# Z2PackDev/TBmodels

Measured on AMD Instinct MI355X. Metric: k-points/sec (H(k)+eig) at N_orb=64, N_R=4096, higher is better.
Workload: dtype f64; 1 GPU; cfg2: dense N_orb=64 N_R=4096, 100000 random k-points per GPU, eigenval (H(k)+eig); kpoints_per_gpu=100000, collective=none, rccl_ranks=0, eigensolver=auto

## Files before the change

### include/tbk.h

```cpp
#ifndef TBK_H
#define TBK_H

#include <stdint.h>

#ifdef __cplusplus
extern "C" {
#endif

typedef struct tbk_model tbk_model;
typedef struct tbk_kdotp tbk_kdotp;
typedef struct tbk_comm tbk_comm;

typedef enum tbk_status {
    TBK_OK = 0,
    TBK_ERR_ARGUMENT = 1,
    TBK_ERR_DEVICE = 2,
    TBK_ERR_MEMORY = 3,
    TBK_ERR_NOT_FINITE = 4,
    TBK_ERR_NO_CONVERGENCE = 5
} tbk_status;

enum { TBK_EIG_AUTO = 0, TBK_EIG_WAVE = 1, TBK_EIG_ROCSOLVER = 2 };
enum {
    TBK_OPT_EIGENSOLVER = 1,
    TBK_OPT_K_CHUNK = 2,
    TBK_OPT_TIMING = 3,
    TBK_OPT_FOLD = 4
};

const char* tbk_version(void);
const char* tbk_last_error(void);
int tbk_device_count(int* count);


int tbk_model_create_dense(int device, int dim, int n_orb, int64_t n_r, const int32_t* R,
                           const double* hop, tbk_model** out);

int tbk_model_create_csr(int device, int dim, int n_orb, int64_t n_r, const int32_t* R,
                         const int64_t* r_ptr, const int32_t* row, const int32_t* col,
                         const double* val, tbk_model** out);

void tbk_model_destroy(tbk_model* m);
int tbk_model_set_option(tbk_model* m, int option, int64_t value);
int tbk_model_info(const tbk_model* m, int* device, int* dim, int* n_orb, int64_t* n_r,
                   int* is_sparse, int64_t* staged_bytes);
enum { TBK_CNT_EIGENVAL_CALLS = 0, TBK_CNT_FOLDED_CALLS = 1, TBK_CNT_FOLDED_KPOINTS = 2,
       TBK_CNT_LIBRARY_CALLS = 3,
       TBK_CNT_COUNT = 4 };
int tbk_model_counter(tbk_model* m, int counter, int64_t* value);


int tbk_hamilton(tbk_model* m, const double* k, int64_t nk, int convention, const double* pos,
                 double* H_out);

int tbk_eigenval(tbk_model* m, const double* k, int64_t nk, double* E_out);

int tbk_eigenval_multi(tbk_model* const* handles, int n_handles, const double* k, int64_t nk, double* E_out);
int tbk_hamilton_multi(tbk_model* const* handles, int n_handles, const double* k, int64_t nk, int convention,
                       const double* pos, double* H_out);

int tbk_hamilton_device(tbk_model* m, const double* d_k, int64_t nk, int convention,
                        const double* d_pos, double* d_H);
int tbk_eigenval_device(tbk_model* m, const double* d_k, int64_t nk, double* d_E);
int tbk_eigenval_device_hint(tbk_model* m, const double* d_k, const double* h_k, int64_t nk, double* d_E);
int tbk_eigenval_check(tbk_model* m);
int tbk_synchronize(tbk_model* m);

enum { TBK_REDUCE_AUTO = 0, TBK_REDUCE_ONE_STAGE = 1, TBK_REDUCE_TWO_STAGE = 2 };
int tbk_tridiagonal_reduce(int device, int n_orb, int64_t nk, const double* H, int method, double* d, double* e,
                           double* H_reduced);

int tbk_reduce_standalone(int device, int n_orb, int64_t nk, int reps, double* us_per_matrix);

int tbk_kdotp_create(int device, int dim, int n_orb, int64_t n_p, const int32_t* powers,
                     const double* coeffs, tbk_kdotp** out);
void tbk_kdotp_destroy(tbk_kdotp* m);
int tbk_kdotp_hamilton(tbk_kdotp* m, const double* k, int64_t nk, double* H_out);
int tbk_kdotp_eigenval(tbk_kdotp* m, const double* k, int64_t nk, double* E_out);
int tbk_kdotp_eigenval_multi(tbk_kdotp* const* handles, int n_handles, const double* k, int64_t nk, double* E_out);
int tbk_kdotp_hamilton_multi(tbk_kdotp* const* handles, int n_handles, const double* k, int64_t nk, double* H_out);

int tbk_kdotp_coefficients(tbk_model* m, const double* k0, int64_t n_p, const int32_t* powers,
                           const double* prefactor, double* coeffs_out);

int tbk_device_malloc(int device, int64_t bytes, void** d_ptr);
int tbk_device_free(int device, void* d_ptr);
int tbk_memcpy_h2d(int device, void* d_dst, const void* h_src, int64_t bytes);
int tbk_memcpy_d2h(int device, void* h_dst, const void* d_src, int64_t bytes);
int tbk_device_mem_info(int device, int64_t* free_bytes, int64_t* total_bytes);

enum { TBK_T_PHASE = 0, TBK_T_HK = 1, TBK_T_EIG = 2, TBK_T_QL = 3, TBK_T_COUNT = 4 };
int tbk_get_timing(tbk_model* m, double* ms, int64_t* launches, int reset);

int tbk_comm_unique_id(void* id128);
int tbk_comm_create(int device, int world_size, int rank, const void* id128, tbk_comm** out);
void tbk_comm_destroy(tbk_comm* c);
int tbk_comm_ranks(tbk_comm* c, int* count, int* rank);
int tbk_comm_allgather_f64(tbk_comm* c, tbk_model* m, const double* d_send, double* d_recv,
                           int64_t count);
int tbk_comm_allgather_f64_overlapped(tbk_comm* c, tbk_model* m, const double* d_send, double* d_recv,
                                      int64_t count, int slot);
int tbk_comm_wait_slot(tbk_comm* c, tbk_model* m, int slot);
int tbk_comm_synchronize(tbk_comm* c);
int tbk_comm_agree(tbk_comm* c, int status, double* verdict);
int tbk_comm_prepare_gather(tbk_comm* c, int n_orb, int64_t per);

int tbk_eigenval_device_gather(tbk_comm* c, tbk_model* m, const double* d_k, const double* h_k, int64_t nk, int64_t per,
                               int host_status, double* d_all, double* d_status_all);

int tbk_mfma_f64_peak(int device, double* tflops);

#ifdef __cplusplus
}
#endif
#endif
```

### tbmodels_amd/_lib.py

```python

import ctypes
import os

import numpy as np

_HERE = os.path.dirname(os.path.abspath(__file__))
LIB_PATH = os.environ.get("TBK_LIBTBK") or os.path.join(_HERE, "libtbk.so")

TBK_OK = 0
TBK_ERR_ARGUMENT = 1
TBK_ERR_DEVICE = 2
TBK_ERR_MEMORY = 3
TBK_ERR_NOT_FINITE = 4
TBK_ERR_NO_CONVERGENCE = 5

TBK_EIG_AUTO, TBK_EIG_WAVE, TBK_EIG_ROCSOLVER = 0, 1, 2
TBK_OPT_EIGENSOLVER, TBK_OPT_K_CHUNK, TBK_OPT_TIMING, TBK_OPT_FOLD = 1, 2, 3, 4
TBK_REDUCE_AUTO, TBK_REDUCE_ONE_STAGE, TBK_REDUCE_TWO_STAGE = 0, 1, 2
TBK_CNT_EIGENVAL_CALLS, TBK_CNT_FOLDED_CALLS, TBK_CNT_FOLDED_KPOINTS, TBK_CNT_LIBRARY_CALLS = 0, 1, 2, 3
TBK_T_PHASE, TBK_T_HK, TBK_T_EIG, TBK_T_QL, TBK_T_COUNT = 0, 1, 2, 3, 4
STAGE_NAMES = ("phase", "hk", "eig", "ql")

_c_int = ctypes.c_int
_c_i64 = ctypes.c_int64
_vp = ctypes.c_void_p
_pp = ctypes.POINTER(ctypes.c_void_p)

SIGNATURES = {
    "tbk_version": (ctypes.c_char_p, []),
    "tbk_last_error": (ctypes.c_char_p, []),
    "tbk_device_count": (_c_int, [ctypes.POINTER(_c_int)]),
    "tbk_model_create_dense": (_c_int, [_c_int, _c_int, _c_int, _c_i64, _vp, _vp, _pp]),
    "tbk_model_create_csr": (_c_int, [_c_int, _c_int, _c_int, _c_i64, _vp, _vp, _vp, _vp, _vp, _pp]),
    "tbk_model_destroy": (None, [_vp]),
    "tbk_model_set_option": (_c_int, [_vp, _c_int, _c_i64]),
    "tbk_model_info": (
        _c_int,
        [_vp, ctypes.POINTER(_c_int), ctypes.POINTER(_c_int), ctypes.POINTER(_c_int), ctypes.POINTER(_c_i64),
         ctypes.POINTER(_c_int), ctypes.POINTER(_c_i64)],
    ),
    "tbk_hamilton": (_c_int, [_vp, _vp, _c_i64, _c_int, _vp, _vp]),
    "tbk_eigenval": (_c_int, [_vp, _vp, _c_i64, _vp]),
    "tbk_eigenval_multi": (_c_int, [_vp, _c_int, _vp, _c_i64, _vp]),
    "tbk_hamilton_multi": (_c_int, [_vp, _c_int, _vp, _c_i64, _c_int, _vp, _vp]),
    "tbk_hamilton_device": (_c_int, [_vp, _vp, _c_i64, _c_int, _vp, _vp]),
    "tbk_eigenval_device": (_c_int, [_vp, _vp, _c_i64, _vp]),
    "tbk_eigenval_device_hint": (_c_int, [_vp, _vp, _vp, _c_i64, _vp]),
    "tbk_model_counter": (_c_int, [_vp, _c_int, ctypes.POINTER(_c_i64)]),
    "tbk_eigenval_check": (_c_int, [_vp]),
    "tbk_synchronize": (_c_int, [_vp]),
    "tbk_tridiagonal_reduce": (_c_int, [_c_int, _c_int, _c_i64, _vp, _c_int, _vp, _vp, _vp]),
    "tbk_reduce_standalone": (_c_int, [_c_int, _c_int, _c_i64, _c_int, ctypes.POINTER(ctypes.c_double)]),
    "tbk_kdotp_create": (_c_int, [_c_int, _c_int, _c_int, _c_i64, _vp, _vp, _pp]),
    "tbk_kdotp_destroy": (None, [_vp]),
    "tbk_kdotp_hamilton": (_c_int, [_vp, _vp, _c_i64, _vp]),
    "tbk_kdotp_eigenval": (_c_int, [_vp, _vp, _c_i64, _vp]),
    "tbk_kdotp_eigenval_multi": (_c_int, [_vp, _c_int, _vp, _c_i64, _vp]),
    "tbk_kdotp_hamilton_multi": (_c_int, [_vp, _c_int, _vp, _c_i64, _vp]),
    "tbk_kdotp_coefficients": (_c_int, [_vp, _vp, _c_i64, _vp, _vp, _vp]),
    "tbk_device_malloc": (_c_int, [_c_int, _c_i64, _pp]),
    "tbk_device_free": (_c_int, [_c_int, _vp]),
    "tbk_memcpy_h2d": (_c_int, [_c_int, _vp, _vp, _c_i64]),
    "tbk_memcpy_d2h": (_c_int, [_c_int, _vp, _vp, _c_i64]),
    "tbk_device_mem_info": (_c_int, [_c_int, ctypes.POINTER(_c_i64), ctypes.POINTER(_c_i64)]),
    "tbk_get_timing": (_c_int, [_vp, ctypes.POINTER(ctypes.c_double), ctypes.POINTER(_c_i64), _c_int]),
    "tbk_comm_unique_id": (_c_int, [_vp]),
    "tbk_comm_create": (_c_int, [_c_int, _c_int, _c_int, _vp, _pp]),
    "tbk_comm_destroy": (None, [_vp]),
    "tbk_comm_ranks": (_c_int, [_vp, ctypes.POINTER(_c_int), ctypes.POINTER(_c_int)]),
    "tbk_comm_allgather_f64": (_c_int, [_vp, _vp, _vp, _vp, _c_i64]),
    "tbk_comm_allgather_f64_overlapped": (_c_int, [_vp, _vp, _vp, _vp, _c_i64, _c_int]),
    "tbk_comm_wait_slot": (_c_int, [_vp, _vp, _c_int]),
    "tbk_comm_synchronize": (_c_int, [_vp]),
    "tbk_comm_agree": (_c_int, [_vp, _c_int, _vp]),
    "tbk_comm_prepare_gather": (_c_int, [_vp, _c_int, _c_i64]),
    "tbk_eigenval_device_gather": (_c_int, [_vp, _vp, _vp, _vp, _c_i64, _c_i64, _c_int, _vp, _vp]),
    "tbk_mfma_f64_peak": (_c_int, [_c_int, ctypes.POINTER(ctypes.c_double)]),
}

_LIB = None


class TbkLibraryError(RuntimeError):
    """``libtbk.so`` is missing or cannot be loaded: the product path has no CPU fallback."""


def lib():
    global _LIB
    if _LIB is None:
        if not os.path.exists(LIB_PATH):
            raise TbkLibraryError(
                "{} not found: build it with `python -c 'import __graft_entry__ as g; g.build()'` "
                "(or `make -C tbmodels_amd/csrc`). There is no CPU fallback.".format(LIB_PATH)
            )
        try:
            handle = ctypes.CDLL(LIB_PATH, mode=ctypes.RTLD_GLOBAL)
        except OSError as exc:
            raise TbkLibraryError("cannot load {}: {}".format(LIB_PATH, exc)) from exc
        for name, (restype, argtypes) in SIGNATURES.items():
            func = getattr(handle, name)
            func.restype = restype
            func.argtypes = argtypes
        _LIB = handle
    return _LIB


def last_error():
    msg = lib().tbk_last_error()
    return msg.decode("utf-8", "replace") if msg else ""


def check(status):
    if status == TBK_OK:
        return
    msg = last_error()
    if status in (TBK_ERR_ARGUMENT, TBK_ERR_NOT_FINITE):
        raise ValueError(msg)
    if status == TBK_ERR_MEMORY:
        raise MemoryError(msg)
    if status == TBK_ERR_NO_CONVERGENCE:
        raise np.linalg.LinAlgError(msg)
    raise RuntimeError(msg)


def ptr(array):
    if array is None:
        return None
    assert array.flags.c_contiguous
    return array.__array_interface__["data"][0]


def device_count():
    count = ctypes.c_int(0)
    check(lib().tbk_device_count(ctypes.byref(count)))
    return count.value
```

### tbmodels_amd/csrc/tbk_api.hip

```cpp

#include <algorithm>
#include <cmath>
#include <cstdarg>
#include <cstdlib>
#include <cstring>
#include <dlfcn.h>
#include <functional>
#include <new>
#include <vector>

#include "tbk_internal.h"

static thread_local char g_err[1024] = "";

void tbk_set_error(const char* fmt, ...) {
    va_list ap;
    va_start(ap, fmt);
    vsnprintf(g_err, sizeof(g_err), fmt, ap);
    va_end(ap);
}

extern "C" const char* tbk_last_error(void) { return g_err; }
extern "C" const char* tbk_version(void) { return "tbk 0.1 (gfx950)"; }

extern "C" int tbk_device_count(int* count) {
    TBK_ARG(count != nullptr, "count is NULL");
    int n = 0;
    hipError_t e = hipGetDeviceCount(&n);
    if (e != hipSuccess) {
        (void)hipGetLastError();
        n = 0;
    }
    *count = n;
    return TBK_OK;
}

int DevBuf::reserve(size_t want) {
    if (want <= bytes) return TBK_OK;
    release();
    const size_t rounded = (want + (size_t(1) << 20) - 1) & ~((size_t(1) << 20) - 1);
    TBK_HIP(hipMalloc(&ptr, rounded));
    bytes = rounded;
    return TBK_OK;
}

void DevBuf::release() {
    if (ptr) (void)hipFree(ptr);
    ptr = nullptr;
    bytes = 0;
}

namespace {
struct RoctxApi {
    int (*push)(const char*) = nullptr;
    int (*pop)() = nullptr;
};
const RoctxApi& roctx_api() {
    static const RoctxApi api = [] {
        RoctxApi a;
        for (const char* name : {"librocprofiler-sdk-roctx.so", "librocprofiler-sdk-roctx.so.1", "libroctx64.so"}) {
            void* h = dlopen(name, RTLD_LAZY | RTLD_GLOBAL);
            if (!h) continue;
            a.push = reinterpret_cast<int (*)(const char*)>(dlsym(h, "roctxRangePushA"));
            a.pop = reinterpret_cast<int (*)()>(dlsym(h, "roctxRangePop"));
            if (a.push && a.pop) break;
            a.push = nullptr;
            a.pop = nullptr;
        }
        return a;
    }();
    return api;
}
const char* const kStageNames[TBK_T_COUNT] = {"tbk:phase_rows", "tbk:hk_contraction", "tbk:tridiag_reduction",
                                              "tbk:tridiag_eigenvalues"};
}

void tbk_range_push(const char* name) {
    const RoctxApi& api = roctx_api();
    if (api.push) (void)api.push(name);
}

void tbk_range_pop() {
    const RoctxApi& api = roctx_api();
    if (api.pop) (void)api.pop();
}

StageTimer::StageTimer(tbk_model* m_, int stage, hipStream_t s)
    : m(m_), on(m_->timing), stream(s ? s : m_->stream) {
    ev.stage = stage;
    if (on) {
        if (hipEventCreate(&ev.start) != hipSuccess || hipEventCreate(&ev.stop) != hipSuccess) {
            on = false;
            return;
        }
        tbk_range_push(kStageNames[stage]);
        (void)hipEventRecord(ev.start, stream);
    }
}

StageTimer::~StageTimer() {
    if (on) {
        (void)hipEventRecord(ev.stop, stream);
        tbk_range_pop();
        m->events.push_back(ev);
    }
}

static inline int64_t round_up(int64_t x, int64_t q) { return (x + q - 1) / q * q; }

static int require_device(int device) {
    int n = 0;
    if (hipGetDeviceCount(&n) != hipSuccess || n == 0) {
        (void)hipGetLastError();
        tbk_set_error("no HIP device visible: libtbk has no CPU path");
        return TBK_ERR_DEVICE;
    }
    if (device < 0 || device >= n) {
        tbk_set_error("device %d out of range (have %d)", device, n);
        return TBK_ERR_ARGUMENT;
    }
    TBK_HIP(hipSetDevice(device));
    return TBK_OK;
}

static int create_common(int device, int dim, int n_orb, int64_t n_r, const int32_t* R,
                         int64_t k_rows_per_r, bool pair_diagonal, tbk_model** out) {
    TBK_ARG(out != nullptr, "out is NULL");
    *out = nullptr;
    TBK_ARG(dim >= 1 && dim <= TBK_MAX_DIM, "dim must be in [1, 8]");
    TBK_ARG(n_orb >= 1 && n_orb <= 32768, "n_orb must be in [1, 32768]");
    TBK_ARG(n_r >= 0 && n_r < (int64_t(1) << 28), "n_r out of range");
    TBK_ARG(n_r == 0 || R != nullptr || k_rows_per_r == 1, "R is NULL");
    TBK_CHECK(require_device(device));

    tbk_model* m = new (std::nothrow) tbk_model();
    if (!m) {
        tbk_set_error("out of host memory");
        return TBK_ERR_MEMORY;
    }
    m->device = device;
    {
        int cus = 0;
        if (hipDeviceGetAttribute(&cus, hipDeviceAttributeMultiprocessorCount, device) == hipSuccess && cus > 0) m->n_cu = cus;
    }
    m->dim = dim;
    m->n_orb = n_orb;
    m->n_r = n_r;
    m->k2 = round_up(n_r * k_rows_per_r, TBK_BK);
    m->n_r_pad = m->k2 / k_rows_per_r;
    m->ncol = (int)(pair_diagonal ? (int64_t)n_orb * (n_orb - 1) / 2 + (n_orb + 1) / 2 : (int64_t)n_orb * (n_orb + 1) / 2);
    m->ncol_pad = (int)round_up(m->ncol, TBK_BNP);

    int rc = TBK_OK;
    auto fail = [&](int code) {
        tbk_model_destroy(m);
        return code;
    };
#define TBK_TRY(expr)                           \
    do {                                        \
        rc = [&]() -> int {                     \
            expr;                               \
            return TBK_OK;                      \
        }();                                    \
        if (rc != TBK_OK) return fail(rc);      \
    } while (0)

    TBK_TRY(TBK_HIP(hipStreamCreateWithFlags(&m->stream, hipStreamNonBlocking)));
    TBK_TRY(TBK_HIP(hipStreamCreateWithFlags(&m->stream_eig, hipStreamNonBlocking)));
    TBK_TRY(TBK_HIP(hipStreamCreateWithFlags(&m->stream_ql, hipStreamNonBlocking)));
    for (int b = 0; b < 2; ++b) {
        TBK_TRY(TBK_HIP(hipEventCreateWithFlags(&m->ev_hk[b], hipEventDisableTiming)));
        TBK_TRY(TBK_HIP(hipEventCreateWithFlags(&m->ev_tri[b], hipEventDisableTiming)));
        TBK_TRY(TBK_HIP(hipEventCreateWithFlags(&m->ev_ql[b], hipEventDisableTiming)));
        TBK_TRY(TBK_HIP(hipEventCreateWithFlags(&m->ev_out[b], hipEventDisableTiming)));
        if (b == 0) TBK_TRY(TBK_HIP(hipEventCreateWithFlags(&m->ev_sync, hipEventDisableTiming | hipEventReleaseToSystem)));
    }
    TBK_TRY(TBK_ROCBLAS(rocblas_create_handle(&m->blas)));
    TBK_TRY(TBK_ROCBLAS(rocblas_set_stream(m->blas, m->stream)));
    TBK_TRY(TBK_CHECK(m->ws_flag.reserve(2 * sizeof(int))));
    TBK_TRY(TBK_HIP(hipMemsetAsync(m->ws_flag.ptr, 0, 2 * sizeof(int), m->stream)));
    m->h_stage_bytes = std::max<size_t>(size_t(320) << 10,
                                        n_orb <= 1024 ? (size_t)n_orb * n_orb * 16 + (size_t)n_orb * dim * 8 + (size_t(64) << 10) : 0);
    if (hipHostMalloc(&m->h_stage, m->h_stage_bytes, hipHostMallocNonCoherent) != hipSuccess) {
        (void)hipGetLastError();
        m->h_stage = nullptr;
        m->h_stage_bytes = 0;
    }

    {
        std::vector<int32_t> colmap((size_t)m->ncol_pad, -1);
        size_t e = 0;
        for (int i = 0; i < n_orb; ++i) {
            if (!pair_diagonal)
                colmap[e++] = (int32_t)((i << 16) | i);
            else if (i % 2 == 0)
                colmap[e++] = i + 1 < n_orb ? (int32_t)((i << 16) | TBK_SLOT_PAIR | (i + 1)) : (int32_t)((i << 16) | i);
            for (int j = i + 1; j < n_orb; ++j) colmap[e++] = (int32_t)((i << 16) | j);
        }
        TBK_TRY(TBK_HIP(hipMalloc((void**)&m->d_colmap, colmap.size() * sizeof(int32_t))));
        TBK_TRY(TBK_HIP(hipMemcpy(m->d_colmap, colmap.data(), colmap.size() * sizeof(int32_t),
                                  hipMemcpyHostToDevice)));
        m->staged_bytes += (int64_t)(colmap.size() * sizeof(int32_t));
    }
    if (n_r > 0 && R != nullptr && k_rows_per_r == 2) m->h_R.assign(R, R + (size_t)n_r * dim);
    if (m->n_r_pad > 0 && R != nullptr) {
        std::vector<int32_t> r_pad((size_t)m->n_r_pad * dim, 0);
        std::memcpy(r_pad.data(), R, (size_t)n_r * dim * sizeof(int32_t));
        TBK_TRY(TBK_HIP(hipMalloc((void**)&m->d_R, r_pad.size() * sizeof(int32_t))));
        TBK_TRY(TBK_HIP(hipMemcpy(m->d_R, r_pad.data(), r_pad.size() * sizeof(int32_t),
                                  hipMemcpyHostToDevice)));
        m->staged_bytes += (int64_t)(r_pad.size() * sizeof(int32_t));
    }
#undef TBK_TRY
    *out = m;
    return TBK_OK;
}

extern "C" int tbk_model_create_dense(int device, int dim, int n_orb, int64_t n_r, const int32_t* R,
                                      const double* hop, tbk_model** out) {
    TBK_ARG(out != nullptr, "out is NULL");
    *out = nullptr;
    TBK_ARG(n_r == 0 || hop != nullptr, "hop is NULL");
    tbk_model* m = nullptr;
    TBK_CHECK(create_common(device, dim, n_orb, n_r, R, 2, true, &m));
    m->sparse = false;
    int rc = TBK_OK;
    double* d_raw = nullptr;
    const size_t raw_bytes = (size_t)n_r * n_orb * n_orb * 2 * sizeof(double);
    rc = [&]() -> int {
        if (raw_bytes) {
            TBK_HIP(hipMalloc((void**)&d_raw, raw_bytes));
            TBK_HIP(hipMemcpyAsync(d_raw, hop, raw_bytes, hipMemcpyHostToDevice, m->stream));
        }
        TBK_CHECK(tbk_stage_dense(m, d_raw));
        TBK_HIP(hipStreamSynchronize(m->stream));
        return TBK_OK;
    }();
    if (d_raw) (void)hipFree(d_raw);
    if (rc != TBK_OK) {
        tbk_model_destroy(m);
        return rc;
    }
    *out = m;
    return TBK_OK;
}

extern "C" int tbk_model_create_csr(int device, int dim, int n_orb, int64_t n_r, const int32_t* R,
                                    const int64_t* r_ptr, const int32_t* row, const int32_t* col,
                                    const double* val, tbk_model** out) {
    TBK_ARG(out != nullptr, "out is NULL");
    *out = nullptr;
    TBK_ARG(n_r >= 0, "n_r out of range");
    TBK_ARG(n_r == 0 || r_ptr != nullptr, "r_ptr is NULL");
    const int64_t nnz = n_r > 0 ? r_ptr[n_r] : 0;
    TBK_ARG(n_r == 0 || r_ptr[0] == 0, "r_ptr[0] must be 0");
    TBK_ARG(nnz >= 0, "negative nnz");
    TBK_ARG(nnz == 0 || (row && col && val), "row/col/val is NULL");
    for (int64_t r = 0; r < n_r; ++r) TBK_ARG(r_ptr[r] <= r_ptr[r + 1], "r_ptr not monotone");
    for (int64_t t = 0; t < nnz; ++t)
        TBK_ARG(row[t] >= 0 && row[t] < n_orb && col[t] >= 0 && col[t] < n_orb,
                "row/col index out of range");

    tbk_model* m = nullptr;
    TBK_CHECK(create_common(device, dim, n_orb, n_r, R, 2, false, &m));
    m->sparse = true;

    auto packed_index = [n_orb](int i, int j) -> int64_t {
        return (int64_t)i * n_orb - (int64_t)i * (i - 1) / 2 + (j - i);
    };
    std::vector<int64_t> cptr((size_t)m->ncol + 1, 0);
    for (int64_t t = 0; t < nnz; ++t) {
        const int i = std::min(row[t], col[t]), j = std::max(row[t], col[t]);
        cptr[(size_t)packed_index(i, j) + 1]++;
    }
    for (int e = 0; e < m->ncol; ++e) cptr[(size_t)e + 1] += cptr[(size_t)e];
    std::vector<int32_t> rec_r((size_t)nnz);
    std::vector<double> rec_v((size_t)nnz * 2);
    {
        std::vector<int64_t> cursor(cptr.begin(), cptr.end() - 1);
        for (int64_t r = 0; r < n_r; ++r)
            for (int64_t t = r_ptr[r]; t < r_ptr[r + 1]; ++t) {
                const int i = row[t], j = col[t];
                const int kind = (i == j) ? 2 : (i < j ? 0 : 1);
                const int64_t e = packed_index(std::min(i, j), std::max(i, j));
                const int64_t slot = cursor[(size_t)e]++;
                rec_r[(size_t)slot] = (int32_t)((kind << 28) | (int32_t)r);
                rec_v[(size_t)slot * 2] = val[2 * t];
                rec_v[(size_t)slot * 2 + 1] = val[2 * t + 1];
            }
    }
    m->nnz_rec = nnz;
    int rc = [&]() -> int {
        TBK_HIP(hipMalloc((void**)&m->d_cptr, cptr.size() * sizeof(int64_t)));
        TBK_HIP(hipMemcpy(m->d_cptr, cptr.data(), cptr.size() * sizeof(int64_t), hipMemcpyHostToDevice));
        m->staged_bytes += (int64_t)(cptr.size() * sizeof(int64_t));
        if (nnz > 0) {
            TBK_HIP(hipMalloc((void**)&m->d_rec_r, (size_t)nnz * sizeof(int32_t)));
            TBK_HIP(hipMalloc((void**)&m->d_rec_v, (size_t)nnz * 2 * sizeof(double)));
            TBK_HIP(hipMemcpy(m->d_rec_r, rec_r.data(), (size_t)nnz * sizeof(int32_t), hipMemcpyHostToDevice));
            TBK_HIP(hipMemcpy(m->d_rec_v, rec_v.data(), (size_t)nnz * 2 * sizeof(double), hipMemcpyHostToDevice));
            m->staged_bytes += nnz * (int64_t)(sizeof(int32_t) + 2 * sizeof(double));
            const int kt = tbk_csr_tile_kpoints(n_r);
            if (kt > 0) {
                std::vector<int64_t> sptr;
                std::vector<int32_t> srec_r;
                std::vector<double> srec_v;
                tbk_csr_schedule(m->ncol, kt, cptr, rec_r, rec_v, sptr, srec_r, srec_v);
                m->sched_steps = sptr.back();
                auto upload = [&](void** dst, const void* src, size_t bytes) -> int {
                    TBK_HIP(hipMalloc(dst, std::max<size_t>(bytes, 8)));
                    if (bytes) TBK_HIP(hipMemcpy(*dst, src, bytes, hipMemcpyHostToDevice));
                    m->staged_bytes += (int64_t)bytes;
                    return TBK_OK;
                };
                TBK_CHECK(upload((void**)&m->d_sptr, sptr.data(), sptr.size() * sizeof(int64_t)));
                TBK_CHECK(upload((void**)&m->d_srec_r, srec_r.data(), srec_r.size() * sizeof(int32_t)));
                TBK_CHECK(upload((void**)&m->d_srec_v, srec_v.data(), srec_v.size() * sizeof(double)));
                m->sched_kt = kt;
            }
        }
        return TBK_OK;
    }();
    if (rc != TBK_OK) {
        tbk_model_destroy(m);
        return rc;
    }
    *out = m;
    return TBK_OK;
}

extern "C" void tbk_model_destroy(tbk_model* m) {
    if (!m) return;
    (void)hipSetDevice(m->device);
    hipStream_t streams[] = {m->stream, m->stream_eig, m->stream_ql, m->stream_xl[0], m->stream_xl[1], m->stream_xl[2]};
    for (hipStream_t st : streams)
        if (st) (void)hipStreamSynchronize(st);
    for (hipEvent_t e : m->ev_xl)
        if (e) (void)hipEventDestroy(e);
    for (int b = 0; b < 2; ++b) {
        if (m->ev_hk[b]) (void)hipEventDestroy(m->ev_hk[b]);
        if (m->ev_tri[b]) (void)hipEventDestroy(m->ev_tri[b]);
        if (m->ev_ql[b]) (void)hipEventDestroy(m->ev_ql[b]);
        if (m->ev_out[b]) (void)hipEventDestroy(m->ev_out[b]);
        if (b == 0 && m->ev_sync) (void)hipEventDestroy(m->ev_sync);
    }
    for (auto& ev : m->events) {
        (void)hipEventDestroy(ev.start);
        (void)hipEventDestroy(ev.stop);
    }
    if (m->blas) (void)rocblas_destroy_handle(m->blas);
    if (m->h_stage) (void)hipHostFree(m->h_stage);
    for (hipStream_t st : streams)
        if (st) (void)hipStreamDestroy(st);
    void* ptrs[] = {m->d_R, m->d_colmap, m->d_B, m->d_cptr, m->d_rec_r, m->d_rec_v, m->d_powers, m->d_sptr, m->d_srec_r, m->d_srec_v};
    for (void* p : ptrs)
        if (p) (void)hipFree(p);
    DevBuf* bufs[] = {&m->ws_phase, &m->ws_H, &m->ws_E,   &m->ws_E2,
                      &m->ws_info,  &m->ws_k, &m->ws_pos, &m->ws_out, &m->ws_out2, &m->ws_flag, &m->ws_orb, &m->ws_part, &m->ws_kfold, &m->ws_kline, &m->ws_band, &m->ws_bandmat[0], &m->ws_bandmat[1], &m->ws_H2, &m->ws_xl, &m->ws_posraw};
    for (DevBuf* b : bufs) b->release();
    tbk_fold_release(m);
    delete m;
}

extern "C" int tbk_model_set_option(tbk_model* m, int option, int64_t value) {
    TBK_ARG(m != nullptr, "model is NULL");
    TBK_LOCK(m);
    switch (option) {
        case TBK_OPT_EIGENSOLVER:
            TBK_ARG(value >= TBK_EIG_AUTO && value <= TBK_EIG_ROCSOLVER, "unknown eigensolver");
            m->eigensolver = (int)value;
            return TBK_OK;
        case TBK_OPT_K_CHUNK:
            TBK_ARG(value >= 0, "k chunk must be >= 0");
            m->k_chunk = value;
            return TBK_OK;
        case TBK_OPT_TIMING:
            m->timing = value != 0;
            return TBK_OK;
        case TBK_OPT_FOLD:
            m->fold_enabled = value != 0;
            return TBK_OK;
        default:
            tbk_set_error("unknown option %d", option);
            return TBK_ERR_ARGUMENT;
    }
}

extern "C" int tbk_model_info(const tbk_model* m, int* device, int* dim, int* n_orb, int64_t* n_r,
                              int* is_sparse, int64_t* staged_bytes) {
    TBK_ARG(m != nullptr, "model is NULL");
    if (device) *device = m->device;
    if (dim) *dim = m->dim;
    if (n_orb) *n_orb = m->n_orb;
    if (n_r) *n_r = m->n_r;
    if (is_sparse) *is_sparse = m->sparse ? 1 : 0;
    if (staged_bytes) *staged_bytes = m->staged_bytes;
    return TBK_OK;
}

static int64_t choose_chunk(tbk_model* m, int64_t nk, bool with_eig) {
    if (nk <= TBK_BM) return TBK_BM;
    const int64_t n = m->n_orb;
    int64_t per_k = m->k2 * 8 + (with_eig ? n * n * 16 + (int64_t)tbk_eig_scratch_per_k(m) : 0);
    if (per_k < 64) per_k = 64;
    size_t free_b = 0, total_b = 0;
    if (hipMemGetInfo(&free_b, &total_b) != hipSuccess) free_b = size_t(8) << 30;
    free_b += m->ws_H.bytes + m->ws_H2.bytes + m->ws_phase.bytes + m->ws_band.bytes + m->ws_bandmat[0].bytes + m->ws_bandmat[1].bytes +
              m->ws_E.bytes + m->ws_xl.bytes;
    const bool mid = n > 64 && n <= 256;
    int64_t budget = std::min<int64_t>((int64_t)(free_b / 4), int64_t(mid ? 64 : n > 64 ? 24 : 6) << 30);
    int64_t chunk = budget / per_k / TBK_BM * TBK_BM;
    int64_t cap = mid ? 131072 : 32768;
    if (n < 64) cap *= std::min<int64_t>(32, (64 / n) * (64 / n));
    chunk = std::max<int64_t>(TBK_BM, std::min<int64_t>(chunk, cap));
    if (m->k_chunk > 0) chunk = round_up(m->k_chunk, TBK_BM);
    else if (chunk >= 4096) chunk = chunk / 4096 * 4096;
    return std::min(chunk, round_up(nk, TBK_BM));
}

static inline int64_t phase_ld(int64_t nk) { return round_up(nk, TBK_BM); }

static int fill_rows(tbk_model* m, const double* d_k, int64_t nk, int64_t nk_pad, double* d_A) {
    if (m->kdotp)
        return tbk_launch_monomials(m->stream, m->d_powers, m->dim, m->n_r, m->k2, d_k, nk, nk_pad, d_A);
    return tbk_launch_phase(m, d_k, nk, nk_pad, d_A);
}

static int build_h(tbk_model* m, const double* d_A, int64_t nk, int64_t nk_pad, int mode,
                   int convention, const double* d_k, const double* d_pos, double* d_H) {
    if (m->sparse)
        return tbk_launch_hk_csr(m, d_A, nk, nk_pad, mode, convention, d_k, d_pos, d_H);
    return tbk_launch_hk_dense(m, d_A, nk, nk_pad, mode, convention, d_k, d_pos, d_H);
}

extern "C" int tbk_hamilton_device(tbk_model* m, const double* d_k, int64_t nk, int convention,
                                   const double* d_pos, double* d_H) {
    TBK_ARG(m != nullptr, "model is NULL");
    TBK_LOCK(m);
    TBK_ARG(convention == 1 || convention == 2, "convention must be 1 or 2");
    TBK_ARG(nk >= 0, "nk < 0");
    if (nk == 0) return TBK_OK;
    TBK_ARG(d_k && d_H, "k / H is NULL");
    TBK_ARG(convention == 2 || d_pos != nullptr, "convention 1 needs pos");
    TBK_HIP(hipSetDevice(m->device));
    const int64_t chunk = choose_chunk(m, nk, false);
    const size_t nn2 = (size_t)m->n_orb * m->n_orb * 2;
    for (int64_t c0 = 0; c0 < nk; c0 += chunk) {
        const int64_t nkc = std::min(chunk, nk - c0);
        const int64_t nk_pad = phase_ld(nkc);
        TBK_CHECK(m->ws_phase.reserve((size_t)std::max<int64_t>(m->k2, 1) * nk_pad * sizeof(double)));
        double* d_A = m->ws_phase.as<double>();
        const double* kc = d_k + c0 * m->dim;
        const bool own_rows = tbk_hk_inline_phases(m, nkc);
        if (!own_rows) TBK_CHECK(fill_rows(m, kc, nkc, nk_pad, d_A));
        const double* d_orb = nullptr;
        const bool inline_orb = m->h_k_inline != nullptr && m->d_pos_inline != nullptr && nk == 1 && own_rows;
        if (convention == 1 && !inline_orb) {
            TBK_CHECK(m->ws_orb.reserve((size_t)nkc * m->n_orb * 2 * sizeof(double)));
            TBK_CHECK(tbk_launch_orbital_phases(m, kc, d_pos, nkc, m->ws_orb.as<double>()));
            d_orb = m->ws_orb.as<double>();
        }
        TBK_CHECK(build_h(m, own_rows ? nullptr : d_A, nkc, nk_pad, HK_FULL, convention, kc, d_orb, d_H + (size_t)c0 * nn2));
    }
    return TBK_OK;
}

constexpr int64_t TBK_SMALL_CALL = 4096;
constexpr int64_t TBK_SMALL_CALL_PER_ORBITAL = 768;

static int launch_tridiag_eigenvalues(tbk_model* m, hipStream_t s, double* d_de, int64_t nk, double* d_E,
                                      bool beside_ql = false, bool small_call = false, const void* d_band = nullptr) {
    if (d_band) TBK_CHECK(tbk_launch_band_chase(m, s, d_band, nk, d_de));
    if (tbk_eig_small_supported(m->n_orb) && !small_call) return tbk_launch_ql(m, s, d_de, nk, d_E, beside_ql);
    return tbk_launch_bisect(m, s, d_de, nk, d_E);
}

static std::vector<int64_t> chunk_schedule(tbk_model* m, int64_t nk, int64_t chunk) {
    std::vector<int64_t> out;
    const int64_t unit = 4096;
    if (!tbk_eig_small_supported(m->n_orb) || m->k_chunk > 0 || chunk < 2 * unit || nk < 3 * unit) {
        for (int64_t c0 = 0; c0 < nk; c0 += chunk) out.push_back(std::min(chunk, nk - c0));
        return out;
    }
    const int64_t last = unit + nk % unit;
    int64_t rest = nk - last;
    const int64_t n_big = (rest + chunk - 1) / chunk;
    for (int64_t i = 0; i < n_big; ++i) {
        const int64_t share = round_up((rest + (n_big - i) - 1) / (n_big - i), unit);
        const int64_t take = std::min(std::min(share, chunk), rest);
        out.push_back(take);
        rest -= take;
    }
    out.push_back(last);
    return out;
}

using HBuilder = std::function<int(int64_t c0, int64_t nkc, double* d_H)>;

static std::vector<int64_t> run_schedule(const std::vector<int64_t>& runs, int64_t chunk) {
    std::vector<int64_t> out;
    int64_t cur = 0;
    for (size_t r = 0; r + 1 < runs.size(); ++r) {
        int64_t len = runs[r + 1] - runs[r];
        if (cur > 0 && cur + len > chunk) {
            out.push_back(cur);
            cur = 0;
        }
        while (len > chunk) {
            out.push_back(chunk);
            len -= chunk;
        }
        cur += len;
    }
    if (cur > 0) out.push_back(cur);
    return out;
}

static int eigenval_wave_pipeline(tbk_model* m, const double* d_k, int64_t nk, double* d_E, const HBuilder* builder = nullptr,
                                  const std::vector<int64_t>* runs = nullptr) {
    int64_t rows_ready_for = -1;
    const auto prepare_rows = [&](int64_t c0, int64_t nkc) -> int {
        if (tbk_hk_inline_phases(m, nkc)) return TBK_OK;
        const int64_t nk_pad = phase_ld(nkc);
        TBK_CHECK(m->ws_phase.reserve((size_t)std::max<int64_t>(m->k2, 1) * nk_pad * sizeof(double)));
        TBK_CHECK(fill_rows(m, d_k + c0 * m->dim, nkc, nk_pad, m->ws_phase.as<double>()));
        rows_ready_for = c0;
        return TBK_OK;
    };
    const HBuilder direct = [&](int64_t c0, int64_t nkc, double* d_H) -> int {
        const int64_t nk_pad = phase_ld(nkc);
        const double* kc = d_k + c0 * m->dim;
        if (tbk_hk_inline_phases(m, nkc)) return build_h(m, nullptr, nkc, nk_pad, HK_TRI, 2, kc, nullptr, d_H);
        if (rows_ready_for != c0) TBK_CHECK(prepare_rows(c0, nkc));
        return build_h(m, m->ws_phase.as<double>(), nkc, nk_pad, HK_TRI, 2, kc, nullptr, d_H);
    };
    const HBuilder& build = builder ? *builder : direct;
    const int64_t chunk = choose_chunk(m, nk, true);
    const size_t n = (size_t)m->n_orb;
    const size_t nn2 = n * n * 2;
    DevBuf* debuf[2] = {&m->ws_E, &m->ws_E2};
    const std::vector<int64_t> sched =
        (runs != nullptr && m->k_chunk == 0 && nk > chunk) ? run_schedule(*runs, chunk) : chunk_schedule(m, nk, chunk);
    const int64_t n_chunks = (int64_t)sched.size();
    const int64_t max_chunk = *std::max_element(sched.begin(), sched.end());
    const bool small_call = nk <= std::max<int64_t>(TBK_SMALL_CALL, TBK_SMALL_CALL_PER_ORBITAL * (int64_t)m->n_orb);
    TBK_CHECK(m->ws_H.reserve((size_t)max_chunk * nn2 * sizeof(double)));
    for (int b = 0; b < (n_chunks > 1 ? 2 : 1); ++b)
        TBK_CHECK(debuf[b]->reserve((size_t)max_chunk * n * 2 * sizeof(double)));
    double* d_H = m->ws_H.as<double>();
    const bool h_overlap = n_chunks > 2 && builder != nullptr && tbk_eig_small_supported(m->n_orb);
    double* d_Hbuf[2] = {d_H, d_H};
    if (h_overlap) {
        TBK_CHECK(m->ws_H2.reserve((size_t)max_chunk * nn2 * sizeof(double)));
        d_Hbuf[1] = m->ws_H2.as<double>();
    }
    const bool two_stage = !tbk_eig_small_supported(m->n_orb) && tbk_eig_two_stage(m) && n_chunks > 1 && !tbk_band_fused(m->n_orb);
    if (two_stage) {
        TBK_CHECK(m->ws_band.reserve((size_t)max_chunk * tbk_band_scratch_per_matrix(m->n_orb)));
        for (int b = 0; b < 2; ++b) TBK_CHECK(m->ws_bandmat[b].reserve((size_t)max_chunk * tbk_band_bytes_per_matrix(m->n_orb)));
        TBK_CHECK(tbk_band_xl_reserve(m, max_chunk));
    }
    if (n_chunks == 1) {
        double* d_de = debuf[0]->as<double>();
        TBK_CHECK(build(0, nk, d_H));
        if (tbk_eig_small_supported(m->n_orb))
            TBK_CHECK(tbk_launch_tridiag(m, m->stream, d_H, nk, d_de));
        else
            TBK_CHECK(tbk_launch_tridiag_stream(m, m->stream, d_H, nk, d_de));
        TBK_CHECK(launch_tridiag_eigenvalues(m, m->stream, d_de, nk, d_E, false, small_call));
        if (m->chunk_done) {
            TBK_HIP(hipEventRecord(m->ev_ql[0], m->stream));
            TBK_CHECK(m->chunk_done(0, nk, m->ev_ql[0]));
        }
        return TBK_OK;
    }
    int64_t prev_c0 = 0, prev_nkc = 0, c0 = 0;
    for (int64_t c = 0; c < n_chunks; ++c) {
        const int b = (int)(c & 1);
        const int64_t nkc = sched[c];
        double* d_de = debuf[b]->as<double>();
        d_H = d_Hbuf[b];
        if (c >= 1) {
            if (!builder) TBK_CHECK(prepare_rows(c0, nkc));
            if (!h_overlap)
                TBK_HIP(hipStreamWaitEvent(m->stream, m->ev_tri[b ^ 1], 0));
            else if (c >= 2)
                TBK_HIP(hipStreamWaitEvent(m->stream, m->ev_tri[b], 0));
            if (c >= 2 && !h_overlap) TBK_HIP(hipStreamWaitEvent(m->stream, m->ev_ql[b], 0));
        }
        TBK_CHECK(build(c0, nkc, d_H));
        TBK_HIP(hipEventRecord(m->ev_hk[b], m->stream));

        TBK_HIP(hipStreamWaitEvent(m->stream_eig, m->ev_hk[b], 0));
        if (c >= 2 && h_overlap) TBK_HIP(hipStreamWaitEvent(m->stream_eig, m->ev_ql[b], 0));
        if (tbk_eig_small_supported(m->n_orb))
            TBK_CHECK(tbk_launch_tridiag(m, m->stream_eig, d_H, nkc, d_de));
        else if (two_stage)
            TBK_CHECK(tbk_launch_band_reduce(m, m->stream_eig, d_H, nkc, m->ws_band.ptr, m->ws_bandmat[b].ptr));
        else
            TBK_CHECK(tbk_launch_tridiag_stream(m, m->stream_eig, d_H, nkc, d_de));
        TBK_HIP(hipEventRecord(m->ev_tri[b], m->stream_eig));

        if (c >= 1) {
            TBK_HIP(hipStreamWaitEvent(m->stream_ql, m->ev_hk[b], 0));
            if (h_overlap) TBK_HIP(hipStreamWaitEvent(m->stream_ql, m->ev_tri[b ^ 1], 0));
            TBK_CHECK(launch_tridiag_eigenvalues(m, m->stream_ql, debuf[b ^ 1]->as<double>(), prev_nkc,
                                                 d_E + (size_t)prev_c0 * n, false, small_call,
                                                 two_stage ? m->ws_bandmat[b ^ 1].ptr : nullptr));
            TBK_HIP(hipEventRecord(m->ev_ql[b ^ 1], m->stream_ql));
            if (m->chunk_done) TBK_CHECK(m->chunk_done(prev_c0, prev_nkc, m->ev_ql[b ^ 1]));
        }
        prev_c0 = c0;
        prev_nkc = nkc;
        c0 += nkc;
    }
    {
        const int b = (int)((n_chunks - 1) & 1);
        TBK_CHECK(launch_tridiag_eigenvalues(m, m->stream_eig, debuf[b]->as<double>(), prev_nkc,
                                             d_E + (size_t)prev_c0 * n, n_chunks > 1,
                                             small_call || n_chunks > 1, two_stage ? m->ws_bandmat[b].ptr : nullptr));
        TBK_HIP(hipEventRecord(m->ev_ql[b], m->stream_eig));
        if (m->chunk_done) TBK_CHECK(m->chunk_done(prev_c0, prev_nkc, m->ev_ql[b]));
    }
    for (int b = 0; b < (n_chunks > 1 ? 2 : 1); ++b) TBK_HIP(hipStreamWaitEvent(m->stream, m->ev_ql[b], 0));
    TBK_HIP(hipStreamWaitEvent(m->stream, m->ev_tri[(n_chunks - 1) & 1], 0));
    return TBK_OK;
}

static int eigenval_folded(tbk_model* m, const double* d_k, const double* h_k, int64_t nk, double* d_E, bool* done) {
    *done = false;
    if (!m->fold_enabled || m->sparse || m->kdotp || m->dim < 2 || m->n_r < 64 || nk < 1024) return TBK_OK;
    if (h_k == nullptr) return TBK_OK;
    std::vector<int64_t> runs;
    const int f = tbk_fold_choose(m, h_k, nk, runs);
    if (f < 0) return TBK_OK;
    const int dim = m->dim;
    TBK_CHECK(m->ws_kfold.reserve((size_t)nk * (dim - 1) * sizeof(double)));
    double* d_k2 = m->ws_kfold.as<double>();
    TBK_CHECK(tbk_fold_drop_component(m, d_k, dim, f, nk, d_k2));
    const size_t nn2 = (size_t)m->n_orb * m->n_orb * 2;
    const int64_t n_runs = (int64_t)runs.size() - 1;
    const int group = tbk_fold_group_size();
    int64_t group_lo = -1;
    tbk_fold_plan_t& plan1 = m->fold[f];
    std::vector<int> reduced;
    for (int d = 0; d < dim; ++d)
        if (d != f) reduced.push_back(d);

    auto piece_plane = [&](int64_t lo, int64_t hi, double* d_Hp) -> int {
        const int64_t len = hi - lo, nk_pad = phase_ld(len);
        TBK_CHECK(m->ws_phase.reserve((size_t)std::max<int64_t>(m->k2, 1) * nk_pad * sizeof(double)));
        TBK_CHECK(fill_rows(m, d_k2 + lo * (dim - 1), len, nk_pad, m->ws_phase.as<double>()));
        return build_h(m, m->ws_phase.as<double>(), len, nk_pad, HK_TRI, 2, d_k2 + lo * (dim - 1), nullptr, d_Hp);
    };

    struct LineInfo {
        bool ok = false;
        int e2 = -1;
        int64_t L = 0;
        int64_t body = 0;
        int64_t n_lines = 0;
    };
    const int dim1 = dim - 1;
    const int line_cap = 512;
    auto same_line = [&](int64_t a0, int64_t b0, int64_t L, int e2) {
        for (int64_t t = 0; t < L; ++t)
            for (int e = 0; e < dim1; ++e)
                if (e != e2 && h_k[(a0 + t) * dim + reduced[e]] != h_k[(b0 + t) * dim + reduced[e]]) return false;
        return true;
    };
    auto analyse = [&](int64_t lo, int64_t hi) -> LineInfo {
        LineInfo li;
        if (dim1 < 2 || hi - lo < 512) return li;
        int e2 = -1;
        int64_t best_changes = hi - lo;
        for (int e = 0; e < dim1; ++e) {
            int64_t changes = 0;
            for (int64_t i = lo + 1; i < hi; ++i) changes += h_k[i * dim + reduced[e]] != h_k[(i - 1) * dim + reduced[e]];
            if (changes < best_changes) {
                best_changes = changes;
                e2 = e;
            }
        }
        if (e2 < 0 || best_changes < 4) return li;
        const int c2 = reduced[e2];
        std::vector<int64_t> sb(1, lo);
        for (int64_t i = lo + 1; i < hi; ++i)
            if (h_k[i * dim + c2] != h_k[(i - 1) * dim + c2]) sb.push_back(i);
        sb.push_back(hi);
        const size_t n_sub = sb.size() - 1;
        if (n_sub < 6) return li;
        const int64_t L = sb[2] - sb[1];
        if (L < 8 || L > TBK_BM) return li;
        size_t first = (sb[1] - sb[0] == L && same_line(sb[0], sb[1], L, e2)) ? 0 : 1, last = first;
        while (last < n_sub && sb[last + 1] - sb[last] == L && same_line(sb[first], sb[last], L, e2)) ++last;
        li.n_lines = (int64_t)(last - first);
        if (li.n_lines < 4) return li;
        li.ok = true;
        li.e2 = e2;
        li.L = L;
        li.body = sb[first];
        return li;
    };
    auto fold_body = [&](tbk_fold_plan_t& plan2, const LineInfo& li, int64_t a0, int64_t n, int slot0) -> int {
        return tbk_fold_lines(m, plan2, d_k2 + a0 * dim1 + li.e2, li.L * dim1, (int)n, slot0);
    };
    auto contract_lines = [&](tbk_fold_plan_t& plan2, const LineInfo& li, int64_t a0, int64_t n, double* d_Hp) -> int {
        const int64_t row_len = (int64_t)m->ncol_pad * 2;
        tbk_fold_saved_t saved2;
        TBK_CHECK(tbk_fold_enter(m, plan2, 0, saved2));
        int rc = m->ws_kline.reserve((size_t)li.L * std::max(dim1 - 1, 1) * sizeof(double));
        if (rc == TBK_OK) rc = tbk_fold_drop_component(m, d_k2 + a0 * dim1, dim1, li.e2, li.L, m->ws_kline.as<double>());
        if (rc == TBK_OK) rc = m->ws_phase.reserve((size_t)std::max<int64_t>(m->k2, 1) * TBK_BM * sizeof(double));
        if (rc == TBK_OK) rc = fill_rows(m, m->ws_kline.as<double>(), li.L, TBK_BM, m->ws_phase.as<double>());
        if (rc == TBK_OK)
            rc = tbk_launch_hk_dense_lines(m, m->ws_phase.as<double>(), n, (int)li.L, plan2.k2 * row_len, d_Hp);
        tbk_fold_leave(m, saved2);
        return rc;
    };

    auto piece = [&](int64_t lo, int64_t hi, double* d_Hp) -> int {
        const LineInfo li = analyse(lo, hi);
        if (!li.ok) return piece_plane(lo, hi, d_Hp);
        tbk_fold_plan_t* plan2 = nullptr;
        TBK_CHECK(tbk_fold_subplan(m, plan1, li.e2, line_cap, &plan2));
        if (!plan2 || plan2->n_rho * 3 > plan1.n_rho) return piece_plane(lo, hi, d_Hp);

        if (li.body > lo) TBK_CHECK(piece_plane(lo, li.body, d_Hp));
        for (int64_t l0 = 0; l0 < li.n_lines; l0 += line_cap) {
            const int64_t nl = std::min<int64_t>(line_cap, li.n_lines - l0);
            const int64_t a0 = li.body + l0 * li.L;
            TBK_CHECK(fold_body(*plan2, li, a0, nl, 0));
            TBK_CHECK(contract_lines(*plan2, li, a0, nl, d_Hp + (size_t)(a0 - lo) * nn2));
        }
        const int64_t body_end = li.body + li.n_lines * li.L;
        if (body_end < hi) TBK_CHECK(piece_plane(body_end, hi, d_Hp + (size_t)(body_end - lo) * nn2));
        return TBK_OK;
    };

    auto enter_run = [&](size_t r, tbk_fold_saved_t& saved) -> int {
        if (group_lo < 0 || (int64_t)r < group_lo || (int64_t)r >= group_lo + group) {
            group_lo = (int64_t)r;
            const int n_g = (int)std::min<int64_t>(group, n_runs - group_lo);
            double kf[64];
            for (int g = 0; g < n_g; ++g) kf[g] = h_k[runs[(size_t)(group_lo + g)] * dim + f];
            TBK_CHECK(tbk_fold_group(m, plan1, kf, n_g, 0));
        }
        return tbk_fold_enter(m, plan1, (int)((int64_t)r - group_lo), saved);
    };
    auto batched = [&](int64_t c0, int64_t nkc, double* d_H, bool* done) -> int {
        *done = false;
        const size_t r0 = (size_t)(std::upper_bound(runs.begin(), runs.end(), c0) - runs.begin()) - 1;
        if (runs[r0] != c0) return TBK_OK;
        size_t r1 = r0;
        while (r1 + 1 < runs.size() && runs[r1 + 1] <= c0 + nkc) ++r1;
        if (r1 - r0 < 2 || runs[r1] != c0 + nkc) return TBK_OK;
        const LineInfo li0 = analyse(runs[r0], runs[r0 + 1]);
        if (!li0.ok || li0.body != runs[r0] || li0.body + li0.n_lines * li0.L != runs[r0 + 1]) return TBK_OK;
        int64_t total = li0.n_lines;
        for (size_t r = r0 + 1; r < r1; ++r) {
            const LineInfo li = analyse(runs[r], runs[r + 1]);
            if (!li.ok || li.e2 != li0.e2 || li.L != li0.L || li.body != runs[r] ||
                li.body + li.n_lines * li.L != runs[r + 1] || !same_line(runs[r0], runs[r], li0.L, li0.e2))
                return TBK_OK;
            total += li.n_lines;
        }
        if (total > line_cap) return TBK_OK;
        tbk_fold_plan_t* plan2 = nullptr;
        TBK_CHECK(tbk_fold_subplan(m, plan1, li0.e2, line_cap, &plan2));
        if (!plan2 || plan2->n_rho * 3 > plan1.n_rho) return TBK_OK;
        int slot = 0;
        for (size_t r = r0; r < r1; ++r) {
            tbk_fold_saved_t saved;
            TBK_CHECK(enter_run(r, saved));
            const int64_t n = (runs[r + 1] - runs[r]) / li0.L;
            const int rc = fold_body(*plan2, li0, runs[r], n, slot);
            tbk_fold_leave(m, saved);
            TBK_CHECK(rc);
            slot += (int)n;
        }
        {
            tbk_fold_saved_t saved;
            TBK_CHECK(enter_run(r1 - 1, saved));
            const int rc = contract_lines(*plan2, li0, c0, total, d_H);
            tbk_fold_leave(m, saved);
            TBK_CHECK(rc);
        }
        *done = true;
        return TBK_OK;
    };

    const HBuilder folded = [&](int64_t c0, int64_t nkc, double* d_H) -> int {
        {
            bool done = false;
            TBK_CHECK(batched(c0, nkc, d_H, &done));
            if (done) return TBK_OK;
        }
        size_t r = (size_t)(std::upper_bound(runs.begin(), runs.end(), c0) - runs.begin()) - 1;
        for (int64_t lo = c0; lo < c0 + nkc; ++r) {
            const int64_t hi = std::min(runs[r + 1], c0 + nkc);
            tbk_fold_saved_t saved;
            TBK_CHECK(enter_run(r, saved));
            const int rc = piece(lo, hi, d_H + (size_t)(lo - c0) * nn2);
            tbk_fold_leave(m, saved);
            TBK_CHECK(rc);
            lo = hi;
        }
        return TBK_OK;
    };
    TBK_CHECK(eigenval_wave_pipeline(m, d_k, nk, d_E, &folded, &runs));
    m->counters[TBK_CNT_FOLDED_CALLS] += 1;
    m->counters[TBK_CNT_FOLDED_KPOINTS] += nk;
    *done = true;
    return TBK_OK;
}

static bool eigenval_own_solvers(const tbk_model* m) {
    return m->eigensolver != TBK_EIG_ROCSOLVER &&
           (tbk_eig_small_supported(m->n_orb) || (m->eigensolver == TBK_EIG_AUTO && tbk_eig_stream_supported(m->n_orb)));
}

static int eigenval_device_solve(tbk_model* m, const double* d_k, const double* h_k, int64_t nk, double* d_E) {
    TBK_ARG(m != nullptr, "model is NULL");
    TBK_LOCK(m);
    TBK_ARG(nk >= 0, "nk < 0");
    if (nk == 0) return TBK_OK;
    TBK_ARG(d_k && d_E, "k / E is NULL");
    TBK_HIP(hipSetDevice(m->device));
    m->call_nk = nk;
    m->counters[TBK_CNT_EIGENVAL_CALLS] += 1;
    if (m->eigensolver == TBK_EIG_WAVE && !tbk_eig_small_supported(m->n_orb)) {
        tbk_set_error("TBK_EIG_WAVE handles n_orb <= 64 only (n_orb = %d)", m->n_orb);
        return TBK_ERR_ARGUMENT;
    }
    if (eigenval_own_solvers(m)) {
        bool done = false;
        TBK_CHECK(eigenval_folded(m, d_k, h_k, nk, d_E, &done));
        if (done) return TBK_OK;
        return eigenval_wave_pipeline(m, d_k, nk, d_E);
    }

    int64_t chunk = choose_chunk(m, nk, true);
    const size_t nn2 = (size_t)m->n_orb * m->n_orb * 2;
    chunk = std::max<int64_t>(1, std::min<int64_t>(chunk, (int64_t(1) << 29) / std::max<int64_t>(1, (int64_t)m->n_orb * m->n_orb)));
    m->counters[TBK_CNT_LIBRARY_CALLS] += 1;
    for (int64_t c0 = 0; c0 < nk; c0 += chunk) {
        const int64_t nkc = std::min(chunk, nk - c0);
        const int64_t nk_pad = phase_ld(nkc);
        TBK_CHECK(m->ws_phase.reserve((size_t)std::max<int64_t>(m->k2, 1) * nk_pad * sizeof(double)));
        TBK_CHECK(m->ws_H.reserve((size_t)nkc * nn2 * sizeof(double)));
        double* d_A = m->ws_phase.as<double>();
        double* d_H = m->ws_H.as<double>();
        const double* kc = d_k + c0 * m->dim;
        TBK_CHECK(fill_rows(m, kc, nkc, nk_pad, d_A));
        TBK_CHECK(build_h(m, d_A, nkc, nk_pad, HK_TRI, 2, kc, nullptr, d_H));
        TBK_CHECK(tbk_eig_batched(m, d_H, nkc, d_E + (size_t)c0 * m->n_orb));
    }
    return TBK_OK;
}

__global__ void __launch_bounds__(256) flag_nonfinite_kernel(const double* __restrict__ E, int64_t total, int* __restrict__ flag) {
    bool bad = false;
    for (int64_t i = (int64_t)blockIdx.x * 256 + threadIdx.x; i < total; i += (int64_t)gridDim.x * 256) bad |= !isfinite(E[i]);
    if (__any(bad) && (threadIdx.x & 63) == 0) atomicAdd(flag, 1);
}

static int eigenval_device_impl(tbk_model* m, const double* d_k, const double* h_k, int64_t nk, double* d_E) {
    TBK_CHECK(eigenval_device_solve(m, d_k, h_k, nk, d_E));
    const bool own_solvers = m != nullptr && eigenval_own_solvers(m);
    if (nk > 0 && m != nullptr && !own_solvers) {
        const int64_t total = nk * m->n_orb;
        const unsigned blocks = (unsigned)std::min<int64_t>((total + 255) / 256, 8 * 1024);
        hipLaunchKernelGGL(flag_nonfinite_kernel, dim3(blocks), dim3(256), 0, m->stream, d_E, total, m->ws_flag.as<int>() + 1);
        TBK_HIP(hipGetLastError());
    }
    return TBK_OK;
}

extern "C" int tbk_eigenval_device(tbk_model* m, const double* d_k, int64_t nk, double* d_E) {
    return eigenval_device_impl(m, d_k, nullptr, nk, d_E);
}

extern "C" int tbk_eigenval_device_hint(tbk_model* m, const double* d_k, const double* h_k, int64_t nk, double* d_E) {
    return eigenval_device_impl(m, d_k, h_k, nk, d_E);
}

extern "C" int tbk_model_counter(tbk_model* m, int counter, int64_t* value) {
    TBK_ARG(m != nullptr && value != nullptr, "model / value is NULL");
    TBK_ARG(counter >= 0 && counter < TBK_CNT_COUNT, "unknown counter");
    TBK_LOCK(m);
    *value = m->counters[counter];
    return TBK_OK;
}

static int wait_main_stream(tbk_model* m) {
    TBK_HIP(hipEventRecord(m->ev_sync, m->stream));
    TBK_HIP(hipEventSynchronize(m->ev_sync));
    return TBK_OK;
}

extern "C" int tbk_synchronize(tbk_model* m) {
    TBK_ARG(m != nullptr, "model is NULL");
    TBK_LOCK(m);
    TBK_HIP(hipSetDevice(m->device));
    return wait_main_stream(m);
}

extern "C" int tbk_eigenval_check(tbk_model* m) {
    TBK_ARG(m != nullptr, "model is NULL");
    TBK_LOCK(m);
    TBK_HIP(hipSetDevice(m->device));
    int flag[2] = {0, 0};
    TBK_HIP(hipMemcpyAsync(flag, m->ws_flag.ptr, sizeof(flag), hipMemcpyDeviceToHost, m->stream));
    TBK_HIP(hipMemsetAsync(m->ws_flag.ptr, 0, sizeof(flag), m->stream));
    TBK_CHECK(wait_main_stream(m));
    if (flag[1] != 0) {
        tbk_set_error("array must not contain infs or NaNs");
        return TBK_ERR_NOT_FINITE;
    }
    if (flag[0] != 0) {
        tbk_set_error("eigensolver did not converge for %d matrices", flag[0]);
        return TBK_ERR_NO_CONVERGENCE;
    }
    return TBK_OK;
}

extern "C" int tbk_hamilton(tbk_model* m, const double* k, int64_t nk, int convention,
                            const double* pos, double* H_out) {
    TBK_ARG(m != nullptr, "model is NULL");
    TBK_LOCK(m);
    TBK_ARG(convention == 1 || convention == 2, "convention must be 1 or 2");
    TBK_ARG(nk >= 0, "nk < 0");
    if (nk == 0) return TBK_OK;
    TBK_ARG(k && H_out, "k / H is NULL");
    TBK_ARG(convention == 2 || pos != nullptr, "convention 1 needs pos");
    TBK_HIP(hipSetDevice(m->device));
    const size_t nn2 = (size_t)m->n_orb * m->n_orb * 2;
    {
        const size_t k_bytes = (size_t)nk * m->dim * sizeof(double), h_bytes = (size_t)nk * nn2 * sizeof(double);
        const size_t p_bytes = convention == 1 ? (size_t)m->n_orb * m->dim * sizeof(double) : 0;
        const size_t h_off = (k_bytes + p_bytes + 63) / 64 * 64;
        if (m->h_stage != nullptr && h_off + h_bytes <= m->h_stage_bytes) {
            char* st = static_cast<char*>(m->h_stage);
            TBK_CHECK(m->ws_k.reserve(k_bytes));
            TBK_CHECK(m->ws_out.reserve(h_bytes));
            const bool inline_k = nk == 1 && !m->sparse && !m->kdotp && tbk_hk_inline_phases(m, 1);
            const double* d_pos = nullptr;
            if (inline_k) {
                if (convention == 1) {
                    const size_t n_pos = (size_t)m->n_orb * m->dim;
                    if (m->pos_cache.size() != n_pos || std::memcmp(m->pos_cache.data(), pos, p_bytes) != 0) {
                        TBK_CHECK(m->ws_posraw.reserve(p_bytes));
                        std::memcpy(st + k_bytes, pos, p_bytes);
                        TBK_HIP(hipMemcpyAsync(m->ws_posraw.ptr, st + k_bytes, p_bytes, hipMemcpyHostToDevice, m->stream));
                        m->pos_cache.assign(pos, pos + n_pos);
                    }
                    m->d_pos_inline = m->ws_posraw.as<double>();
                    d_pos = m->d_pos_inline;
                }
                m->h_k_inline = k;
            } else {
                std::memcpy(st, k, k_bytes);
                TBK_HIP(hipMemcpyAsync(m->ws_k.ptr, st, k_bytes, hipMemcpyHostToDevice, m->stream));
                if (convention == 1) {
                    TBK_CHECK(m->ws_pos.reserve(p_bytes));
                    std::memcpy(st + k_bytes, pos, p_bytes);
                    TBK_HIP(hipMemcpyAsync(m->ws_pos.ptr, st + k_bytes, p_bytes, hipMemcpyHostToDevice, m->stream));
                    d_pos = m->ws_pos.as<double>();
                }
            }
            constexpr size_t ZERO_COPY_MAX = size_t(1) << 20;
            const bool direct = h_bytes <= ZERO_COPY_MAX;
            double* d_out = direct ? reinterpret_cast<double*>(st + h_off) : m->ws_out.as<double>();
            const int rc_inline = tbk_hamilton_device(m, m->ws_k.as<double>(), nk, convention, d_pos, d_out);
            m->h_k_inline = nullptr;
            m->d_pos_inline = nullptr;
            TBK_CHECK(rc_inline);
            if (!direct) TBK_HIP(hipMemcpyAsync(st + h_off, m->ws_out.ptr, h_bytes, hipMemcpyDeviceToHost, m->stream));
            TBK_CHECK(wait_main_stream(m));
            std::memcpy(H_out, st + h_off, h_bytes);
            return TBK_OK;
        }
    }
    const size_t total_bytes = (size_t)nk * nn2 * sizeof(double);
    const size_t chunk_bytes = std::min<size_t>(size_t(128) << 20, std::max<size_t>(size_t(16) << 20, total_bytes / 4));
    int64_t out_chunk = std::max<int64_t>(1, (int64_t)(chunk_bytes / (nn2 * sizeof(double))));
    out_chunk = std::min(out_chunk, nk);
    const int64_t n_chunks = (nk + out_chunk - 1) / out_chunk;
    TBK_CHECK(m->ws_k.reserve((size_t)nk * m->dim * sizeof(double)));
    TBK_HIP(hipMemcpyAsync(m->ws_k.ptr, k, (size_t)nk * m->dim * sizeof(double), hipMemcpyHostToDevice, m->stream));
    const double* d_pos = nullptr;
    if (convention == 1) {
        TBK_CHECK(m->ws_pos.reserve((size_t)m->n_orb * m->dim * sizeof(double)));
        TBK_HIP(hipMemcpyAsync(m->ws_pos.ptr, pos, (size_t)m->n_orb * m->dim * sizeof(double),
                               hipMemcpyHostToDevice, m->stream));
        d_pos = m->ws_pos.as<double>();
    }
    DevBuf* obuf[2] = {&m->ws_out, &m->ws_out2};
    for (int b = 0; b < (n_chunks > 1 ? 2 : 1); ++b) TBK_CHECK(obuf[b]->reserve((size_t)out_chunk * nn2 * sizeof(double)));
    auto compute = [&](int64_t c) -> int {
        const int64_t c0 = c * out_chunk, nkc = std::min(out_chunk, nk - c0);
        TBK_CHECK(tbk_hamilton_device(m, m->ws_k.as<double>() + c0 * m->dim, nkc, convention, d_pos, obuf[c & 1]->as<double>()));
        TBK_HIP(hipEventRecord(m->ev_out[c & 1], m->stream));
        return TBK_OK;
    };
    TBK_CHECK(compute(0));
    for (int64_t c = 0; c < n_chunks; ++c) {
        const int64_t c0 = c * out_chunk, nkc = std::min(out_chunk, nk - c0);
        if (c + 1 < n_chunks) TBK_CHECK(compute(c + 1));
        TBK_HIP(hipEventSynchronize(m->ev_out[c & 1]));
        TBK_HIP(hipMemcpy(H_out + (size_t)c0 * nn2, obuf[c & 1]->ptr, (size_t)nkc * nn2 * sizeof(double), hipMemcpyDeviceToHost));
    }
    return wait_main_stream(m);
}

__global__ void __launch_bounds__(256) export_small_kernel(const double* __restrict__ E, int64_t count, const int* __restrict__ flag,
                                                           double* __restrict__ host_E, int* __restrict__ host_flag) {
    for (int64_t i = (int64_t)blockIdx.x * 256 + threadIdx.x; i < count; i += (int64_t)gridDim.x * 256) host_E[i] = E[i];
    if (blockIdx.x == 0 && threadIdx.x < 2) host_flag[threadIdx.x] = flag[threadIdx.x];
}

extern "C" int tbk_eigenval(tbk_model* m, const double* k, int64_t nk, double* E_out) {
    TBK_ARG(m != nullptr, "model is NULL");
    TBK_LOCK(m);
    TBK_ARG(nk >= 0, "nk < 0");
    if (nk == 0) return TBK_OK;
    TBK_ARG(k && E_out, "k / E is NULL");
    TBK_HIP(hipSetDevice(m->device));
    const size_t k_bytes = (size_t)nk * m->dim * sizeof(double), e_bytes = (size_t)nk * m->n_orb * sizeof(double);
    TBK_CHECK(m->ws_k.reserve(k_bytes));
    TBK_CHECK(m->ws_out.reserve(e_bytes));
    const size_t e_off = (k_bytes + 63) / 64 * 64;
    if (m->h_stage != nullptr && e_off + e_bytes + 16 <= m->h_stage_bytes) {
        char* st = static_cast<char*>(m->h_stage);
        int* flag = reinterpret_cast<int*>(st + e_off + e_bytes);
        const bool inline_k = nk == 1 && !m->sparse && !m->kdotp && eigenval_own_solvers(m) && tbk_hk_inline_phases(m, 1);
        if (inline_k) {
            m->h_k_inline = k;
        } else {
            std::memcpy(st, k, k_bytes);
            TBK_HIP(hipMemcpyAsync(m->ws_k.ptr, st, k_bytes, hipMemcpyHostToDevice, m->stream));
        }
        const int rc_inline = eigenval_device_impl(m, m->ws_k.as<double>(), k, nk, m->ws_out.as<double>());
        m->h_k_inline = nullptr;
        TBK_CHECK(rc_inline);
        {
            const int64_t count = nk * m->n_orb;
            const unsigned blocks = (unsigned)std::min<int64_t>((count + 255) / 256, 64);
            hipLaunchKernelGGL(export_small_kernel, dim3(blocks), dim3(256), 0, m->stream, m->ws_out.as<double>(), count,
                               m->ws_flag.as<int>(), reinterpret_cast<double*>(st + e_off), flag);
            TBK_HIP(hipGetLastError());
        }
        TBK_CHECK(wait_main_stream(m));
        std::memcpy(E_out, st + e_off, e_bytes);
        if (flag[0] != 0 || flag[1] != 0) return tbk_eigenval_check(m);
        return TBK_OK;
    }
    TBK_HIP(hipMemcpyAsync(m->ws_k.ptr, k, k_bytes, hipMemcpyHostToDevice, m->stream));
    TBK_CHECK(eigenval_device_impl(m, m->ws_k.as<double>(), k, nk, m->ws_out.as<double>()));
    TBK_HIP(hipMemcpyAsync(E_out, m->ws_out.ptr, e_bytes, hipMemcpyDeviceToHost, m->stream));
    return tbk_eigenval_check(m);
}

extern "C" int tbk_tridiagonal_reduce(int device, int n_orb, int64_t nk, const double* H, int method, double* d, double* e,
                                      double* H_reduced) {
    TBK_ARG(nk >= 0, "nk < 0");
    TBK_ARG(n_orb >= 1 && (n_orb <= 64 || tbk_eig_stream_supported(n_orb)),
            "n_orb must be in [1, 4096] (larger matrices go through rocSOLVER as a whole)");
    TBK_ARG(method >= TBK_REDUCE_AUTO && method <= TBK_REDUCE_TWO_STAGE, "unknown reduction method");
    TBK_ARG(method != TBK_REDUCE_TWO_STAGE || tbk_eig_band_supported(n_orb), "the two-stage reduction handles 64 < n_orb <= 4096");
    TBK_ARG(method != TBK_REDUCE_ONE_STAGE || n_orb <= 512, "the one-stage reduction handles n_orb <= 512");
    if (nk == 0) return TBK_OK;
    TBK_ARG(H && d && e, "H / d / e is NULL");
    tbk_model* m = nullptr;
    TBK_CHECK(create_common(device, 1, n_orb, 0, nullptr, 2, false, &m));
    const size_t n = (size_t)n_orb, mat_bytes = n * n * 2 * sizeof(double);
    int rc = [&]() -> int {
        TBK_LOCK(m);
        m->call_nk = nk;
        TBK_CHECK(m->ws_H.reserve((size_t)nk * mat_bytes));
        TBK_CHECK(m->ws_E.reserve((size_t)nk * n * 2 * sizeof(double)));
        TBK_HIP(hipMemcpyAsync(m->ws_H.ptr, H, (size_t)nk * mat_bytes, hipMemcpyHostToDevice, m->stream));
        if (tbk_eig_small_supported(n_orb))
            TBK_CHECK(tbk_launch_tridiag(m, m->stream, m->ws_H.as<double>(), nk, m->ws_E.as<double>()));
        else
            TBK_CHECK(tbk_launch_tridiag_stream(m, m->stream, m->ws_H.as<double>(), nk, m->ws_E.as<double>(), method));
        TBK_HIP(hipMemcpyAsync(d, m->ws_E.ptr, (size_t)nk * n * sizeof(double), hipMemcpyDeviceToHost, m->stream));
        TBK_HIP(hipMemcpyAsync(e, m->ws_E.as<double>() + (size_t)nk * n, (size_t)nk * n * sizeof(double), hipMemcpyDeviceToHost,
                               m->stream));
        if (H_reduced)
            TBK_HIP(hipMemcpyAsync(H_reduced, m->ws_H.ptr, (size_t)nk * mat_bytes, hipMemcpyDeviceToHost, m->stream));
        TBK_HIP(hipStreamSynchronize(m->stream));
        return TBK_OK;
    }();
    tbk_model_destroy(m);
    return rc;
}

__global__ void __launch_bounds__(256) random_hermitian_kernel(double* __restrict__ H, int n, int64_t nk) {
    const int64_t total = nk * (int64_t)n * n;
    for (int64_t t = (int64_t)blockIdx.x * 256 + threadIdx.x; t < total; t += (int64_t)gridDim.x * 256) {
        const int64_t mat = t / ((int64_t)n * n);
        const int r = (int)((t / n) % n), c = (int)(t % n);
        const int i = r < c ? r : c, j = r < c ? c : r;
        uint64_t x = (uint64_t)mat * 0x9E3779B97F4A7C15ull + (uint64_t)i * 0xBF58476D1CE4E5B9ull + (uint64_t)j * 0x94D049BB133111EBull + 1;
        x ^= x >> 30; x *= 0xBF58476D1CE4E5B9ull; x ^= x >> 27; x *= 0x94D049BB133111EBull; x ^= x >> 31;
        const double re = (double)(int64_t)(x >> 11) * (1.0 / 9007199254740992.0) - 0.5;
        x ^= x >> 29; x *= 0x9E3779B97F4A7C15ull; x ^= x >> 32;
        const double im = (double)(int64_t)(x >> 11) * (1.0 / 9007199254740992.0) - 0.5;
        H[2 * t] = re;
        H[2 * t + 1] = i == j ? 0.0 : (r < c ? im : -im);
    }
}

extern "C" int tbk_reduce_standalone(int device, int n_orb, int64_t nk, int reps, double* us_per_matrix) {
    TBK_ARG(us_per_matrix != nullptr, "us_per_matrix is NULL");
    TBK_ARG(nk >= 1 && reps >= 1, "nk / reps < 1");
    TBK_ARG(n_orb >= 1 && (n_orb <= 64 || tbk_eig_stream_supported(n_orb)), "n_orb must be in [1, 4096]");
    for (int q = 0; q < 3; ++q) us_per_matrix[q] = 0.0;
    tbk_model* m = nullptr;
    TBK_CHECK(create_common(device, 1, n_orb, 0, nullptr, 2, false, &m));
    const size_t n = (size_t)n_orb, mat_bytes = n * n * 2 * sizeof(double);
    DevBuf pristine;
    hipEvent_t ev[2] = {nullptr, nullptr};
    int rc = [&]() -> int {
        TBK_LOCK(m);
        m->call_nk = nk;
        TBK_CHECK(pristine.reserve((size_t)nk * mat_bytes));
        TBK_CHECK(m->ws_H.reserve((size_t)nk * mat_bytes));
        TBK_CHECK(m->ws_E.reserve((size_t)nk * n * 2 * sizeof(double)));
        TBK_HIP(hipEventCreate(&ev[0]));
        TBK_HIP(hipEventCreate(&ev[1]));
        hipLaunchKernelGGL(random_hermitian_kernel, dim3(4096), dim3(256), 0, m->stream, pristine.as<double>(), n_orb, nk);
        TBK_HIP(hipGetLastError());
        const bool band = !tbk_eig_small_supported(n_orb) && tbk_eig_two_stage(m);
        if (band) {
            TBK_CHECK(m->ws_band.reserve((size_t)nk * tbk_band_scratch_per_matrix(n_orb)));
            TBK_CHECK(m->ws_bandmat[0].reserve((size_t)nk * tbk_band_bytes_per_matrix(n_orb)));
        }
        for (int what = 0; what < (band ? 3 : 1); ++what) {
            float sum = 0.0f;
            for (int r = 0; r <= reps; ++r) {
                if (what != 2)
                    TBK_HIP(hipMemcpyAsync(m->ws_H.ptr, pristine.ptr, (size_t)nk * mat_bytes, hipMemcpyDeviceToDevice, m->stream));
                TBK_HIP(hipEventRecord(ev[0], m->stream));
                if (what == 0) {
                    if (tbk_eig_small_supported(n_orb))
                        TBK_CHECK(tbk_launch_tridiag(m, m->stream, m->ws_H.as<double>(), nk, m->ws_E.as<double>()));
                    else
                        TBK_CHECK(tbk_launch_tridiag_stream(m, m->stream, m->ws_H.as<double>(), nk, m->ws_E.as<double>(), TBK_REDUCE_AUTO));
                } else if (what == 1) {
                    TBK_CHECK(tbk_launch_band_reduce(m, m->stream, m->ws_H.as<double>(), nk, m->ws_band.ptr, m->ws_bandmat[0].ptr));
                } else {
                    TBK_CHECK(tbk_launch_band_chase(m, m->stream, m->ws_bandmat[0].ptr, nk, m->ws_E.as<double>()));
                }
                TBK_HIP(hipEventRecord(ev[1], m->stream));
                TBK_HIP(hipEventSynchronize(ev[1]));
                float ms = 0.0f;
                TBK_HIP(hipEventElapsedTime(&ms, ev[0], ev[1]));
                if (r > 0) sum += ms;
            }
            us_per_matrix[what] = (double)sum / reps * 1e3 / (double)nk;
        }
        return TBK_OK;
    }();
    for (auto& e : ev)
        if (e) (void)hipEventDestroy(e);
    pristine.release();
    tbk_model_destroy(m);
    return rc;
}

extern "C" int tbk_kdotp_create(int device, int dim, int n_orb, int64_t n_p, const int32_t* powers,
                                const double* coeffs, tbk_kdotp** out) {
    TBK_ARG(out != nullptr, "out is NULL");
    *out = nullptr;
    TBK_ARG(n_p == 0 || (powers && coeffs), "powers / coeffs is NULL");
    for (int64_t t = 0; t < n_p * dim; ++t) TBK_ARG(powers[t] >= 0, "negative power");
    tbk_model* m = nullptr;
    TBK_CHECK(create_common(device, dim, n_orb, n_p, nullptr, 1, false, &m));
    m->kdotp = true;
    double* d_raw = nullptr;
    const size_t raw_bytes = (size_t)n_p * n_orb * n_orb * 2 * sizeof(double);
    int rc = [&]() -> int {
        if (n_p > 0) {
            TBK_HIP(hipMalloc((void**)&m->d_powers, (size_t)n_p * dim * sizeof(int32_t)));
            TBK_HIP(hipMemcpy(m->d_powers, powers, (size_t)n_p * dim * sizeof(int32_t), hipMemcpyHostToDevice));
            TBK_HIP(hipMalloc((void**)&d_raw, raw_bytes));
            TBK_HIP(hipMemcpyAsync(d_raw, coeffs, raw_bytes, hipMemcpyHostToDevice, m->stream));
        }
        TBK_CHECK(tbk_stage_kdotp(m, d_raw));
        TBK_HIP(hipStreamSynchronize(m->stream));
        return TBK_OK;
    }();
    if (d_raw) (void)hipFree(d_raw);
    if (rc != TBK_OK) {
        tbk_model_destroy(m);
        return rc;
    }
    tbk_kdotp* kp = new (std::nothrow) tbk_kdotp();
    if (!kp) {
        tbk_model_destroy(m);
        tbk_set_error("out of host memory");
        return TBK_ERR_MEMORY;
    }
    kp->core = m;
    *out = kp;
    return TBK_OK;
}

extern "C" void tbk_kdotp_destroy(tbk_kdotp* kp) {
    if (!kp) return;
    tbk_model_destroy(kp->core);
    delete kp;
}

extern "C" int tbk_kdotp_hamilton(tbk_kdotp* kp, const double* k, int64_t nk, double* H_out) {
    TBK_ARG(kp != nullptr, "model is NULL");
    return tbk_hamilton(kp->core, k, nk, 2, nullptr, H_out);
}

extern "C" int tbk_kdotp_eigenval(tbk_kdotp* kp, const double* k, int64_t nk, double* E_out) {
    TBK_ARG(kp != nullptr, "model is NULL");
    return tbk_eigenval(kp->core, k, nk, E_out);
}

extern "C" int tbk_device_malloc(int device, int64_t bytes, void** d_ptr) {
    TBK_ARG(d_ptr != nullptr && bytes >= 0, "bad malloc arguments");
    TBK_CHECK(require_device(device));
    *d_ptr = nullptr;
    if (bytes == 0) return TBK_OK;
    TBK_HIP(hipMalloc(d_ptr, (size_t)bytes));
    return TBK_OK;
}

extern "C" int tbk_device_free(int device, void* d_ptr) {
    if (!d_ptr) return TBK_OK;
    TBK_CHECK(require_device(device));
    TBK_HIP(hipFree(d_ptr));
    return TBK_OK;
}

extern "C" int tbk_memcpy_h2d(int device, void* d_dst, const void* h_src, int64_t bytes) {
    TBK_CHECK(require_device(device));
    if (bytes > 0) {
        TBK_HIP(hipMemcpy(d_dst, h_src, (size_t)bytes, hipMemcpyHostToDevice));
        TBK_HIP(hipDeviceSynchronize());
    }
    return TBK_OK;
}

extern "C" int tbk_memcpy_d2h(int device, void* h_dst, const void* d_src, int64_t bytes) {
    TBK_CHECK(require_device(device));
    if (bytes > 0) TBK_HIP(hipMemcpy(h_dst, d_src, (size_t)bytes, hipMemcpyDeviceToHost));
    return TBK_OK;
}

extern "C" int tbk_device_mem_info(int device, int64_t* free_bytes, int64_t* total_bytes) {
    TBK_CHECK(require_device(device));
    size_t f = 0, t = 0;
    TBK_HIP(hipMemGetInfo(&f, &t));
    if (free_bytes) *free_bytes = (int64_t)f;
    if (total_bytes) *total_bytes = (int64_t)t;
    return TBK_OK;
}

extern "C" int tbk_get_timing(tbk_model* m, double* ms, int64_t* launches, int reset) {
    TBK_ARG(m != nullptr, "model is NULL");
    TBK_LOCK(m);
    TBK_HIP(hipSetDevice(m->device));
    TBK_HIP(hipStreamSynchronize(m->stream));
    TBK_HIP(hipStreamSynchronize(m->stream_eig));
    TBK_HIP(hipStreamSynchronize(m->stream_ql));
    for (auto& ev : m->events) {
        float t = 0.f;
        if (hipEventElapsedTime(&t, ev.start, ev.stop) == hipSuccess) {
            m->t_ms[ev.stage] += (double)t;
            m->t_n[ev.stage] += 1;
        }
        (void)hipEventDestroy(ev.start);
        (void)hipEventDestroy(ev.stop);
    }
    m->events.clear();
    for (int i = 0; i < TBK_T_COUNT; ++i) {
        if (ms) ms[i] = m->t_ms[i];
        if (launches) launches[i] = m->t_n[i];
        if (reset) {
            m->t_ms[i] = 0.0;
            m->t_n[i] = 0;
        }
    }
    return TBK_OK;
}

extern "C" int tbk_mfma_f64_peak(int device, double* tflops) {
    TBK_ARG(tflops != nullptr, "tflops is NULL");
    TBK_CHECK(require_device(device));
    return tbk_run_mfma_f64_peak(tflops);
}
```

### tbmodels_amd/csrc/tbk_hk_dense.hip

```cpp

#include <algorithm>
#include <cstdlib>
#include <type_traits>

#include "tbk_internal.h"

namespace {

typedef double d4 __attribute__((ext_vector_type(4)));
typedef double d2 __attribute__((ext_vector_type(2)));
typedef __attribute__((address_space(1))) const void* gptr_t;
typedef __attribute__((address_space(3))) void* lptr_t;

constexpr int LDA = TBK_BM + 16;
constexpr int LDB = 2 * TBK_BNP + 16;
constexpr int STAGE_DOUBLES = TBK_BK * (LDA + LDB);

static_assert(TBK_BM == 128 && TBK_BNP == 64 && TBK_BK == 16, "wave decomposition is written for 128x64x16");

struct HkArgs {
    const double* A;
    const double* Bt;
    const int32_t* colmap;
    const double* kpts;
    const int32_t* R;
    int64_t n_r;
    const double* pos;
    double* H;
    int64_t k2;
    int64_t nk;
    int64_t nk_pad;
    int ncol_pad;
    int n_orb;
    int dim;
    int mt_count;
    int nt_count;
    int xcd_rows;
    double* P;
    int splits;
    int unit_grid;
    int64_t p_rows;
    int64_t a_tile_stride;
    int64_t b_tile_stride;
    int rows_per_tile;
    int block_offset;
    int p_tiles;
    int sub_splits;
    double* P2;
    double k_val[TBK_MAX_DIM];
    int k_inline;
    const double* pos_raw;
};

__device__ __forceinline__ double hk_kcomp(const HkArgs& a, int64_t kq, int d) { return a.k_inline ? a.k_val[d] : a.kpts[kq * a.dim + d]; }

template <int MODE, int CONV>
__device__ __forceinline__ void store_element(const HkArgs& a, int64_t kq, int oi, int oj, double re, double im) {
    if (CONV == 1 && oi != oj) {
        d2 ei, ej;
        if (a.k_inline) {
            double di = 0.0, dj = 0.0;
            for (int d = 0; d < a.dim; ++d) {
                di = fma(a.k_val[d], a.pos_raw[oi * a.dim + d], di);
                dj = fma(a.k_val[d], a.pos_raw[oj * a.dim + d], dj);
            }
            double sn, cs;
            sincospi(2.0 * di, &sn, &cs);
            ei = (d2){cs, sn};
            sincospi(2.0 * dj, &sn, &cs);
            ej = (d2){cs, sn};
        } else {
            ei = *reinterpret_cast<const d2*>(a.pos + ((size_t)kq * a.n_orb + oi) * 2);
            ej = *reinterpret_cast<const d2*>(a.pos + ((size_t)kq * a.n_orb + oj) * 2);
        }
        const double cs = ei[0] * ej[0] + ei[1] * ej[1], sn = ei[0] * ej[1] - ei[1] * ej[0];
        const double t = re * cs - im * sn;
        im = re * sn + im * cs;
        re = t;
    }
    double* hk = a.H + (size_t)kq * a.n_orb * a.n_orb * 2;
    *reinterpret_cast<d2*>(hk + ((size_t)oi * a.n_orb + oj) * 2) = (d2){re, im};
    if (MODE == HK_FULL && oi != oj) *reinterpret_cast<d2*>(hk + ((size_t)oj * a.n_orb + oi) * 2) = (d2){re, -im};
}

template <int MODE, int CONV>
__device__ __forceinline__ void store_slot(const HkArgs& a, int64_t kq, int32_t slot, double v0, double v1) {
    const int oi = slot >> 16, oj = slot & 0x7fff;
    if (slot & TBK_SLOT_PAIR) {
        double* hk = a.H + (size_t)kq * a.n_orb * a.n_orb * 2;
        *reinterpret_cast<d2*>(hk + ((size_t)oi * a.n_orb + oi) * 2) = (d2){v0, 0.0};
        *reinterpret_cast<d2*>(hk + ((size_t)oj * a.n_orb + oj) * 2) = (d2){v1, 0.0};
        return;
    }
    store_element<MODE, CONV>(a, kq, oi, oj, v0, v1);
}

__device__ __forceinline__ bool tile_of_block(const HkArgs& a, int b, int& mt, int& nt) {
    if (a.xcd_rows == 0) {
        nt = b % a.nt_count;
        mt = b / a.nt_count;
        return mt < a.mt_count;
    }
    const int x = b & 7;
    const int t = b >> 3;
    const int base = a.mt_count >> 3, extra = a.mt_count & 7;
    const int rows = base + (x < extra ? 1 : 0);
    if (t >= rows * a.nt_count) return false;
    const int start = x * base + (x < extra ? x : extra);
    const int full = rows / a.xcd_rows;
    const int per_group = a.xcd_rows * a.nt_count;
    int row;
    if (t < full * per_group) {
        const int g = t / per_group, r = t % per_group;
        row = g * a.xcd_rows + r % a.xcd_rows;
        nt = r / a.xcd_rows;
    } else {
        const int tt = t - full * per_group, rr = rows - full * a.xcd_rows;
        row = full * a.xcd_rows + tt % rr;
        nt = tt / rr;
    }
    mt = start + row;
    return true;
}

template <int MODE, int CONV, bool SPLIT>
__global__ void __launch_bounds__(256, 2) hk_dense_kernel(const HkArgs a) {
    extern __shared__ __attribute__((aligned(16))) double smem[];

    const int unit = (int)blockIdx.x + a.block_offset;
    const int split_y = SPLIT ? unit / a.unit_grid : 0;
    int mt_idx, nt_idx;
    if (!tile_of_block(a, SPLIT ? unit - split_y * a.unit_grid : unit, mt_idx, nt_idx)) return;

    const int tid = threadIdx.x;
    const int lane = tid & 63;
    const int wave = __builtin_amdgcn_readfirstlane(tid >> 6);
    const int wm = wave >> 1;
    const int wn = wave & 1;
    const int l15 = lane & 15;
    const int l4 = lane >> 4;

    const int64_t m0 = (int64_t)mt_idx * a.rows_per_tile;
    const int64_t n0 = (int64_t)nt_idx * TBK_BNP;

    d4 acc[4][2][2];
#pragma unroll
    for (int i = 0; i < 4; ++i)
#pragma unroll
        for (int j = 0; j < 2; ++j)
#pragma unroll
            for (int p = 0; p < 2; ++p) acc[i][j][p] = (d4){0.0, 0.0, 0.0, 0.0};

    int s_begin = 0, n_stage = (int)(a.k2 / TBK_BK);
    if (SPLIT) {
        const int per = (n_stage + a.splits - 1) / a.splits;
        s_begin = min(split_y * per, n_stage);
        n_stage = min(s_begin + per, n_stage);
        if (a.p_tiles > 0) {
            const int per2 = (n_stage - s_begin + a.sub_splits - 1) / a.sub_splits;
            s_begin = min(s_begin + (int)blockIdx.y * per2, n_stage);
            n_stage = min(s_begin + per2, n_stage);
        }
    }

    const uint32_t lane_bytes = (uint32_t)lane * 16u;
    const int64_t ldgA = a.nk_pad * (int64_t)sizeof(double);
    const int64_t ldgB = (int64_t)a.ncol_pad * 2 * (int64_t)sizeof(double);
    const char* rowA = reinterpret_cast<const char*>(a.A + (int64_t)mt_idx * a.a_tile_stride) + ((int64_t)s_begin * TBK_BK + wave) * ldgA;
    const char* rowB = reinterpret_cast<const char*>(a.Bt + (int64_t)mt_idx * a.b_tile_stride + n0 * 2) + ((int64_t)s_begin * TBK_BK + wave) * ldgB;
    auto issue_stage = [&](auto bufc) {
        constexpr int buf = decltype(bufc)::value;
        double* sA = smem + buf * STAGE_DOUBLES + wave * LDA;
        double* sB = smem + buf * STAGE_DOUBLES + TBK_BK * LDA + wave * LDB;
        uint32_t off = lane_bytes;
        asm volatile("" : "+v"(off));
#pragma unroll
        for (int i = 0; i < 4; ++i) {
            __builtin_amdgcn_global_load_lds((gptr_t)(rowA + (int64_t)(4 * i) * ldgA + off), (lptr_t)(sA + 4 * i * LDA), 16, 0, 0);
            __builtin_amdgcn_global_load_lds((gptr_t)(rowB + (int64_t)(4 * i) * ldgB + off), (lptr_t)(sB + 4 * i * LDB), 16, 0, 0);
        }
        rowA += TBK_BK * ldgA;
        rowB += TBK_BK * ldgB;
    };
    typedef __attribute__((address_space(3))) const double* lds_cptr;
    uint32_t fragA[2][TBK_BK / 4], fragB[2][TBK_BK / 4];
    {
        const uint32_t s0 = (uint32_t)(uintptr_t)(lptr_t)smem;
#pragma unroll
        for (int buf = 0; buf < 2; ++buf)
#pragma unroll
            for (int ks = 0; ks < TBK_BK / 4; ++ks) {
                fragA[buf][ks] = s0 + 8u * (uint32_t)(buf * STAGE_DOUBLES + wm * 64 + l15 + (ks * 4 + l4) * LDA);
                fragB[buf][ks] = s0 + 8u * (uint32_t)(buf * STAGE_DOUBLES + TBK_BK * LDA + wn * 64 + l15 + (ks * 4 + l4) * LDB);
                asm volatile("" : "+v"(fragA[buf][ks]), "+v"(fragB[buf][ks]));
            }
    }
    struct Frags {
        double fa[4], fb[2][2];
    };
    auto read_frags = [&](auto bufc, auto ksc) -> Frags {
        constexpr int buf = decltype(bufc)::value, ks = decltype(ksc)::value;
        const lds_cptr sA = (lds_cptr)(uintptr_t)fragA[buf][ks];
        const lds_cptr sB = (lds_cptr)(uintptr_t)fragB[buf][ks];
        Frags f;
#pragma unroll
        for (int i = 0; i < 4; ++i) f.fa[i] = sA[i * 16];
#pragma unroll
        for (int j = 0; j < 2; ++j) {
            f.fb[j][0] = sB[j * 32];
            f.fb[j][1] = sB[j * 32 + 16];
        }
        return f;
    };
    auto mfma_step = [&](const Frags& f) {
#pragma unroll
        for (int i = 0; i < 4; ++i)
#pragma unroll
            for (int j = 0; j < 2; ++j) {
                acc[i][j][0] = __builtin_amdgcn_mfma_f64_16x16x4f64(f.fa[i], f.fb[j][0], acc[i][j][0], 0, 0, 0);
                acc[i][j][1] = __builtin_amdgcn_mfma_f64_16x16x4f64(f.fa[i], f.fb[j][1], acc[i][j][1], 0, 0, 0);
            }
    };
    using buf0 = std::integral_constant<int, 0>;
    using buf1 = std::integral_constant<int, 1>;
    using ks0 = std::integral_constant<int, 0>;
    using ks1 = std::integral_constant<int, 1>;
    using ks2 = std::integral_constant<int, 2>;
    using ks3 = std::integral_constant<int, 3>;
    static_assert(TBK_BK == 16, "four K steps per stage are written out below");
    auto stage = [&](auto bufc, auto nextc, Frags& cur, bool more) {
        Frags f1 = read_frags(bufc, ks1{});
        mfma_step(cur);
        Frags f2 = read_frags(bufc, ks2{});
        mfma_step(f1);
        Frags f3 = read_frags(bufc, ks3{});
        mfma_step(f2);
        __syncthreads();
        if (more) cur = read_frags(nextc, ks0{});
        mfma_step(f3);
    };

    const int left = n_stage - s_begin;
    if (left > 0) issue_stage(buf0{});
    __syncthreads();
    Frags cur = read_frags(buf0{}, ks0{});
    for (int pair = 0; pair < (left >> 1); ++pair) {
        issue_stage(buf1{});
        stage(buf0{}, buf1{}, cur, true);
        const bool more = 2 * pair + 2 < left;
        if (more) issue_stage(buf0{});
        stage(buf1{}, buf0{}, cur, more);
    }
    if (left & 1) stage(buf0{}, buf1{}, cur, false);

#pragma unroll
    for (int j = 0; j < 2; ++j) {
        const int e = (int)n0 + (wn * 2 + j) * 16 + l15;
        const int32_t ij = a.colmap[e];
        if (ij < 0) continue;
#pragma unroll
        for (int i = 0; i < 4; ++i) {
#pragma unroll
            for (int r = 0; r < 4; ++r) {
                const int local = wm * 64 + i * 16 + l4 + 4 * r;
                const int64_t kq = m0 + local;
                if (local >= a.rows_per_tile || kq >= a.nk) continue;
                if (SPLIT) {
                    double* part =
                        a.p_tiles > 0
                            ? a.P2 + ((((size_t)blockIdx.y * a.p_tiles + blockIdx.x) * TBK_BM + local) * TBK_BNP +
                                      (wn * 2 + j) * 16 + l15) * 2
                            : a.P + (((size_t)split_y * a.p_rows + kq) * a.ncol_pad + e) * 2;
                    *reinterpret_cast<d2*>(part) = (d2){acc[i][j][0][r], acc[i][j][1][r]};
                } else {
                    store_slot<MODE, CONV>(a, kq, ij, acc[i][j][0][r], acc[i][j][1][r]);
                }
            }
        }
    }
}

constexpr int GEMV_U = 8;

template <int NKV, bool INLINE_PHASES>
__global__ void __launch_bounds__(256) hk_gemv_kernel(const HkArgs a, int strip_doubles) {
    extern __shared__ __attribute__((aligned(16))) double s_rows[];
    constexpr int U = NKV >= 32 ? 4 : GEMV_U;
    const int lane = threadIdx.x & 63;
    const int wave = __builtin_amdgcn_readfirstlane(threadIdx.x >> 6);
    const int nblk = a.ncol_pad >> 6;
    const int b = (int)blockIdx.x, n_wg = (int)gridDim.x;
    const int xcd = b & 7, per_xcd = n_wg >> 3, extra = n_wg & 7;
    const int wg = xcd * per_xcd + min(xcd, extra) + (b >> 3);
    const int task = wg * 4 + wave;
    const int sl = task / nblk, cb = task - sl * nblk;
    if (sl >= a.splits) return;
    const int64_t n_pairs = a.k2 >> 1;
    const int64_t kk0 = 2 * (sl * n_pairs / a.splits);
    const int n_rows = (int)(2 * ((sl + 1) * n_pairs / a.splits) - kk0);
    const int64_t kbase = (int64_t)blockIdx.z * NKV;
    const int nk_here = (int)min((int64_t)NKV, a.nk - kbase);
    const int64_t ld2 = a.ncol_pad;
    const d2* rows = reinterpret_cast<const d2*>(a.Bt) + kk0 * ld2 + cb * 64;
    double* strip = s_rows + wave * strip_doubles;

    d2 buf0[U], buf1[U];
    double acc[NKV][2];
#pragma unroll
    for (int q = 0; q < NKV; ++q) acc[q][0] = acc[q][1] = 0.0;

    auto fetch = [&](d2 (&buf)[U], int base) {
#pragma unroll
        for (int u = 0; u < U; ++u) {
            const int r = min(base + u, n_rows - 1);
            buf[u] = __builtin_nontemporal_load(rows + (int64_t)r * ld2 + lane);
        }
    };
    auto consume = [&](const d2 (&buf)[U], int row) {
        const double* arow = INLINE_PHASES ? strip + row * NKV : a.A + (kk0 + row) * a.nk_pad + kbase;
        const int64_t lda = INLINE_PHASES ? NKV : a.nk_pad;
#pragma unroll
        for (int u = 0; u < U; ++u) {
            if (!INLINE_PHASES && row + u >= n_rows) break;
#pragma unroll
            for (int q = 0; q < NKV; ++q) {
                const double aq = arow[u * lda + q];
                acc[q][0] = fma(aq, buf[u][0], acc[q][0]);
                acc[q][1] = fma(aq, buf[u][1], acc[q][1]);
            }
        }
    };
    fetch(buf0, 0);
    fetch(buf1, U);
    if (INLINE_PHASES) {
        for (int idx = lane; idx < ((n_rows + 15) >> 4) * 8 * NKV; idx += 64) {
            const int rr = idx / NKV, q = idx % NKV;
            const int64_t r = (kk0 >> 1) + rr;
            double sn = 0.0, cs = 0.0;
            if (q < nk_here && r < a.n_r && 2 * rr < n_rows) {
                double dot = 0.0;
                for (int d = 0; d < a.dim; ++d) dot = fma(hk_kcomp(a, kbase + q, d), (double)a.R[r * a.dim + d], dot);
                sincospi(2.0 * dot, &sn, &cs);
            }
            strip[(2 * rr) * NKV + q] = cs;
            strip[(2 * rr + 1) * NKV + q] = sn;
        }
        asm volatile("s_waitcnt lgkmcnt(0)" ::: "memory");
    }
    for (int row = 0; row < n_rows; row += 2 * U) {
        consume(buf0, row);
        __builtin_amdgcn_sched_barrier(0);
        fetch(buf0, row + 2 * U);
        __builtin_amdgcn_sched_barrier(0);
        consume(buf1, row + U);
        __builtin_amdgcn_sched_barrier(0);
        fetch(buf1, row + 3 * U);
        __builtin_amdgcn_sched_barrier(0);
    }
    const bool hi = (lane & 8) != 0;
    const int e = cb * 64 + (lane >> 4) * 16 + (lane & 7) * 2 + (hi ? 1 : 0);
#pragma unroll
    for (int q = 0; q < NKV; ++q) {
        const double got = __shfl_xor(hi ? acc[q][0] : acc[q][1], 8, 64);
        if (q < nk_here) {
            double* part = a.P + (((size_t)sl * a.p_rows + kbase + q) * a.ncol_pad + e) * 2;
            *reinterpret_cast<d2*>(part) = hi ? (d2){got, acc[q][1]} : (d2){acc[q][0], got};
        }
    }
}

template <int MODE, int CONV>
__global__ void __launch_bounds__(256) hk_tiny_kernel(const HkArgs a, int strip_doubles) {
    extern __shared__ __attribute__((aligned(16))) double s_tiny[];
    const int lane = threadIdx.x & 63;
    const int wave = __builtin_amdgcn_readfirstlane(threadIdx.x >> 6);
    const int cb = blockIdx.x;
    const int64_t n_pairs = a.k2 >> 1;
    const int64_t kk0 = 2 * (wave * n_pairs / 4);
    const int n_rows = (int)(2 * ((wave + 1) * n_pairs / 4) - kk0);
    const int64_t ld2 = a.ncol_pad;
    const d2* rows = reinterpret_cast<const d2*>(a.Bt) + kk0 * ld2 + cb * 64;
    double* strip = s_tiny + wave * strip_doubles;
    d2* part = reinterpret_cast<d2*>(s_tiny + 4 * strip_doubles);
    d2 buf0[GEMV_U], buf1[GEMV_U];
    auto fetch = [&](d2 (&buf)[GEMV_U], int base) {
#pragma unroll
        for (int u = 0; u < GEMV_U; ++u) buf[u] = rows[(int64_t)min(base + u, n_rows - 1) * ld2 + lane];
    };
    fetch(buf0, 0);
    fetch(buf1, GEMV_U);
    for (int rr = lane; rr < ((n_rows + 15) >> 4) * 8; rr += 64) {
        const int64_t r = (kk0 >> 1) + rr;
        double sn = 0.0, cs = 0.0;
        if (r < a.n_r && 2 * rr < n_rows) {
            double dot = 0.0;
            for (int d = 0; d < a.dim; ++d) dot = fma(hk_kcomp(a, 0, d), (double)a.R[r * a.dim + d], dot);
            sincospi(2.0 * dot, &sn, &cs);
        }
        strip[2 * rr] = cs;
        strip[2 * rr + 1] = sn;
    }
    asm volatile("s_waitcnt lgkmcnt(0)" ::: "memory");
    double acc0 = 0.0, acc1 = 0.0;
    auto consume = [&](const d2 (&buf)[GEMV_U], int row) {
#pragma unroll
        for (int u = 0; u < GEMV_U; ++u) {
            const double aq = strip[row + u];
            acc0 = fma(aq, buf[u][0], acc0);
            acc1 = fma(aq, buf[u][1], acc1);
        }
    };
    for (int row = 0; row < n_rows; row += 2 * GEMV_U) {
        consume(buf0, row);
        __builtin_amdgcn_sched_barrier(0);
        fetch(buf0, row + 2 * GEMV_U);
        __builtin_amdgcn_sched_barrier(0);
        consume(buf1, row + GEMV_U);
        __builtin_amdgcn_sched_barrier(0);
        fetch(buf1, row + 3 * GEMV_U);
        __builtin_amdgcn_sched_barrier(0);
    }
    const bool hi = (lane & 8) != 0;
    const int el = (lane >> 4) * 16 + (lane & 7) * 2 + (hi ? 1 : 0);
    const double got = __shfl_xor(hi ? acc0 : acc1, 8, 64);
    part[wave * 64 + el] = hi ? (d2){got, acc1} : (d2){acc0, got};
    __syncthreads();
    if (wave != 0) return;
    const int e = cb * 64 + lane;
    const int32_t ij = a.colmap[e];
    if (ij < 0) return;
    d2 sum = part[lane];
#pragma unroll
    for (int w = 1; w < 4; ++w) {
        sum[0] += part[w * 64 + lane][0];
        sum[1] += part[w * 64 + lane][1];
    }
    store_slot<MODE, CONV>(a, 0, ij, sum[0], sum[1]);
}

template <int MODE, int CONV>
__global__ void __launch_bounds__(256) hk_finish_kernel(const HkArgs a) {
    const int64_t idx = (int64_t)blockIdx.x * 256 + threadIdx.x;
    const int e = (int)(idx % a.ncol_pad);
    const int64_t kq = idx / a.ncol_pad;
    if (kq >= a.nk) return;
    const int32_t ij = a.colmap[e];
    if (ij < 0) return;
    double re = 0.0, im = 0.0;
    for (int sp = 0; sp < a.splits; ++sp) {
        const d2 v = *reinterpret_cast<const d2*>(a.P + (((size_t)sp * a.p_rows + kq) * a.ncol_pad + e) * 2);
        re += v[0];
        im += v[1];
    }
    store_slot<MODE, CONV>(a, kq, ij, re, im);
}

template <int MODE, int CONV>
__global__ void __launch_bounds__(256) hk_finish_wide_kernel(const HkArgs a) {
    __shared__ double part[4][16][2];
    const int lane = threadIdx.x & 63, wave = threadIdx.x >> 6;
    const int el = lane & 15;
    const int j = wave * 4 + (lane >> 4);
    const int64_t idx = (int64_t)blockIdx.x * 16 + el;
    const int e = (int)(idx % a.ncol_pad);
    const int64_t kq = idx / a.ncol_pad;
    double re = 0.0, im = 0.0;
    if (kq < a.nk)
        for (int sp = j; sp < a.splits; sp += 16) {
            const d2 v = *reinterpret_cast<const d2*>(a.P + (((size_t)sp * a.p_rows + kq) * a.ncol_pad + e) * 2);
            re += v[0];
            im += v[1];
        }
    re += __shfl_xor(re, 16, 64);
    im += __shfl_xor(im, 16, 64);
    re += __shfl_xor(re, 32, 64);
    im += __shfl_xor(im, 32, 64);
    if (lane < 16) {
        part[wave][el][0] = re;
        part[wave][el][1] = im;
    }
    __syncthreads();
    if (threadIdx.x < 16 && kq < a.nk) {
        const int32_t ij = a.colmap[e];
        if (ij < 0) return;
        const double sr = (part[0][el][0] + part[1][el][0]) + (part[2][el][0] + part[3][el][0]);
        const double si = (part[0][el][1] + part[1][el][1]) + (part[2][el][1] + part[3][el][1]);
        store_slot<MODE, CONV>(a, kq, ij, sr, si);
    }
}

template <int MODE, int CONV>
__global__ void __launch_bounds__(256) hk_finish_tiles_kernel(const HkArgs a) {
    const int unit = (int)blockIdx.x + a.block_offset;
    const int split_y = unit / a.unit_grid;
    int mt_idx, nt_idx;
    if (!tile_of_block(a, unit - split_y * a.unit_grid, mt_idx, nt_idx)) return;
    const int el = threadIdx.x & (TBK_BNP - 1);
    const int e = nt_idx * TBK_BNP + el;
    const int32_t ij = a.colmap[e];
    if (ij < 0) return;
    for (int local = threadIdx.x / TBK_BNP; local < a.rows_per_tile; local += 256 / TBK_BNP) {
        const int64_t kq = (int64_t)mt_idx * a.rows_per_tile + local;
        if (kq >= a.nk) break;
        double re = 0.0, im = 0.0;
        for (int sp = 0; sp < a.sub_splits; ++sp) {
            const d2 v = *reinterpret_cast<const d2*>(
                a.P2 + ((((size_t)sp * a.p_tiles + blockIdx.x) * TBK_BM + local) * TBK_BNP + el) * 2);
            re += v[0];
            im += v[1];
        }
        if (a.splits > 1)
            *reinterpret_cast<d2*>(a.P + (((size_t)split_y * a.p_rows + kq) * a.ncol_pad + e) * 2) = (d2){re, im};
        else
            store_slot<MODE, CONV>(a, kq, ij, re, im);
    }
}

template <int MODE, int CONV>
hipError_t launch_gemv(tbk_model* m, const HkArgs& a, size_t lds, hipStream_t s) {
    const int tasks = (a.ncol_pad >> 6) * a.splits;
    const dim3 grid((unsigned)((tasks + 3) / 4), 1, (unsigned)((a.nk + 31) / 32));
    static std::atomic<bool> raised[2][6][TBK_MAX_DEVICES] = {};
#define TBK_GEMV(N, SLOT)                                                                                               \
    do {                                                                                                                \
        if (a.A == nullptr) {                                                                                           \
            hipError_t e1 = tbk_raise_lds_limit(reinterpret_cast<const void*>(&hk_gemv_kernel<N, true>), 160 * 1024, raised[0][SLOT]); \
            if (e1 != hipSuccess) return e1;                                                                            \
            hipLaunchKernelGGL((hk_gemv_kernel<N, true>), grid, dim3(256), lds, s, a, (int)(lds / 32));                                  \
        } else {                                                                                                        \
            hipError_t e1 = tbk_raise_lds_limit(reinterpret_cast<const void*>(&hk_gemv_kernel<N, false>), 160 * 1024, raised[1][SLOT]); \
            if (e1 != hipSuccess) return e1;                                                                            \
            hipLaunchKernelGGL((hk_gemv_kernel<N, false>), grid, dim3(256), lds, s, a, (int)(lds / 32));                                 \
        }                                                                                                               \
    } while (0)
    if (a.nk <= 1)
        TBK_GEMV(1, 0);
    else if (a.nk <= 2)
        TBK_GEMV(2, 1);
    else if (a.nk <= 4)
        TBK_GEMV(4, 2);
    else if (a.nk <= 8)
        TBK_GEMV(8, 3);
    else if (a.nk <= 16)
        TBK_GEMV(16, 4);
    else
        TBK_GEMV(32, 5);
#undef TBK_GEMV
    (void)m;
    hipError_t e = hipGetLastError();
    if (e != hipSuccess) return e;
    const int64_t threads = a.nk * a.ncol_pad;
    if (a.splits >= 32)
        hipLaunchKernelGGL((hk_finish_wide_kernel<MODE, CONV>), dim3((unsigned)((threads + 15) / 16)), dim3(256), 0, s, a);
    else
        hipLaunchKernelGGL((hk_finish_kernel<MODE, CONV>), dim3((unsigned)((threads + 255) / 256)), dim3(256), 0, s, a);
    return hipGetLastError();
}

constexpr int TAIL_MAX_ROUNDS = 12;

template <int MODE, int CONV>
int launch(tbk_model* m, const HkArgs& a0, int grid) {
    hipStream_t s = m->stream;
    const size_t lds = 2 * STAGE_DOUBLES * sizeof(double);
    static std::atomic<bool> raised[TBK_MAX_DEVICES] = {};
    static std::atomic<bool> raised_split[TBK_MAX_DEVICES] = {};
    TBK_HIP(tbk_raise_lds_limit(reinterpret_cast<const void*>(&hk_dense_kernel<MODE, CONV, false>), 160 * 1024, raised));
    TBK_HIP(tbk_raise_lds_limit(reinterpret_cast<const void*>(&hk_dense_kernel<MODE, CONV, true>), 160 * 1024, raised_split));
    HkArgs a = a0;
    a.unit_grid = grid;
    const int slots = 2 * m->n_cu;
    const int n_stage = (int)(a.k2 / TBK_BK);
    const int units = grid * a.splits;
    const int full = units / slots * slots, tail = units - full;
    const int unit_stages = (n_stage + a.splits - 1) / a.splits;
    int sub = 1;
    if (full > 0 && tail > 0 && units < TAIL_MAX_ROUNDS * slots && unit_stages >= 8) {
        auto rounds = [&](int u) { return u <= slots / 2 ? 0.54 : (double)((u + slots - 1) / slots); };
        const double round_ms = 1.97 * unit_stages / 512.0;
        const double plain = rounds(tail) * round_ms;
        double best = std::min(0.9 * plain, plain - 0.03);
        for (int sp = 2; sp <= std::min(64, unit_stages / 4); ++sp) {
            const double cost = rounds(tail * sp) / sp * round_ms + sp * tail * 9e-5 + 0.01;
            if (cost < best) {
                best = cost;
                sub = sp;
            }
        }
    }
    const size_t base_bytes = a.splits > 1 ? (size_t)a.splits * a.p_rows * a.ncol_pad * 2 * sizeof(double) : 0;
    if (sub >= 2) {
        TBK_CHECK(m->ws_part.reserve(base_bytes + (size_t)sub * tail * TBK_BM * TBK_BNP * 2 * sizeof(double)));
        a.P = a.splits > 1 ? m->ws_part.as<double>() : nullptr;
        if (a.splits > 1)
            hipLaunchKernelGGL((hk_dense_kernel<MODE, CONV, true>), dim3(full), dim3(256), lds, s, a);
        else
            hipLaunchKernelGGL((hk_dense_kernel<MODE, CONV, false>), dim3(full), dim3(256), lds, s, a);
        TBK_HIP(hipGetLastError());
        HkArgs t = a;
        t.block_offset = full;
        t.p_tiles = tail;
        t.sub_splits = sub;
        t.P2 = reinterpret_cast<double*>(m->ws_part.as<char>() + base_bytes);
        hipLaunchKernelGGL((hk_dense_kernel<MODE, CONV, true>), dim3(tail, sub), dim3(256), lds, s, t);
        TBK_HIP(hipGetLastError());
        hipLaunchKernelGGL((hk_finish_tiles_kernel<MODE, CONV>), dim3(tail), dim3(256), 0, s, t);
        TBK_HIP(hipGetLastError());
    } else if (a.splits > 1) {
        hipLaunchKernelGGL((hk_dense_kernel<MODE, CONV, true>), dim3(units), dim3(256), lds, s, a);
        TBK_HIP(hipGetLastError());
    } else {
        hipLaunchKernelGGL((hk_dense_kernel<MODE, CONV, false>), dim3(grid), dim3(256), lds, s, a);
        TBK_HIP(hipGetLastError());
    }
    if (a.splits > 1) {
        const int64_t threads = a.nk * a.ncol_pad;
        hipLaunchKernelGGL((hk_finish_kernel<MODE, CONV>), dim3((unsigned)((threads + 255) / 256)), dim3(256), 0, s, a);
        TBK_HIP(hipGetLastError());
    }
    return TBK_OK;
}

int gemv_nkv(int64_t nk) {
    int nkv = 1;
    while (nkv < std::min<int64_t>(nk, 32)) nkv *= 2;
    return nkv;
}
int64_t gemv_strip_rows(const tbk_model* m, int64_t slices) {
    const int64_t n_pairs = m->k2 / 2;
    return (2 * ((n_pairs + slices - 1) / slices) + 15) / 16 * 16;
}

void gemv_plan(const tbk_model* m, int64_t nk, int* slices_out, size_t* lds_out) {
    const int nblk = m->ncol_pad / 64;
    const int64_t n_pairs = m->k2 / 2;
    const size_t per_split = (size_t)nk * m->ncol_pad * 2 * sizeof(double);
    const int64_t cap = std::max<int64_t>(1, (int64_t)((size_t(256) << 20) / per_split));
    const int64_t wave_slots = (int64_t)m->n_cu * 8;
    int64_t slices = wave_slots / nblk;
    size_t lds = 80 * 1024;
    const int64_t rows_one_round = slices > 0 ? (m->k2 + slices - 1) / slices : m->k2 + 1;
    if (slices < 1 || nblk * slices * 10 < wave_slots * 9 || rows_one_round > 384 || slices > cap) {
        slices = std::max<int64_t>(m->k2 / 256, std::min<int64_t>(((int64_t)m->n_cu * 32 + nblk - 1) / nblk, n_pairs / 8));
        slices = std::max<int64_t>(1, std::min(cap, slices));
        lds = 16 * 1024;
    }
    slices = std::max<int64_t>(1, std::min(slices, n_pairs / 8));
    if (nblk * slices * 2 <= wave_slots) lds = 16 * 1024;
    if (lds < 64 * 1024) {
        const size_t need = (size_t)4 * gemv_strip_rows(m, slices) * gemv_nkv(nk) * sizeof(double);
        if (need <= size_t(64) * 1024) lds = std::max(lds, need);
    }
    *slices_out = (int)slices;
    *lds_out = lds;
}

}

bool tbk_hk_inline_phases(const tbk_model* m, int64_t nk) {
    if (!tbk_hk_gemv_path(m, nk) || m->kdotp || m->d_R == nullptr) return false;
    int slices;
    size_t lds;
    gemv_plan(m, nk, &slices, &lds);
    return gemv_strip_rows(m, slices) * gemv_nkv(nk) <= (int64_t)(lds / 32);
}

bool tbk_hk_gemv_path(const tbk_model* m, int64_t nk) {
    if (nk < 1 || m->k2 <= 0 || m->sparse) return false;
    if (nk <= 32) return true;
    return nk <= 4096 && m->ncol_pad <= 256 && m->k2 < 16 * TBK_BK;
}

int tbk_launch_hk_dense(tbk_model* m, const double* d_A, int64_t nk, int64_t nk_pad, int mode,
                        int convention, const double* d_k, const double* d_pos, double* d_H) {
    if (nk == 0) return TBK_OK;
    HkArgs a;
    a.A = d_A;
    a.Bt = m->d_B;
    a.colmap = m->d_colmap;
    a.kpts = d_k;
    a.R = m->d_R;
    a.n_r = m->n_r;
    a.pos = d_pos;
    a.H = d_H;
    a.k2 = m->k2;
    a.nk = nk;
    a.nk_pad = nk_pad;
    a.ncol_pad = m->ncol_pad;
    a.n_orb = m->n_orb;
    a.dim = m->dim;
    a.mt_count = (int)((nk + TBK_BM - 1) / TBK_BM);
    a.nt_count = m->ncol_pad / TBK_BNP;
    int grid;
    if (a.mt_count >= 32) {
        a.xcd_rows = 4;
        const int max_rows = (a.mt_count + 7) / 8;
        grid = max_rows * a.nt_count * 8;
    } else {
        a.xcd_rows = 0;
        grid = a.mt_count * a.nt_count;
    }
    a.P = nullptr;
    a.splits = 1;
    a.p_rows = 0;
    a.a_tile_stride = TBK_BM;
    a.b_tile_stride = 0;
    a.rows_per_tile = TBK_BM;
    a.block_offset = 0;
    a.p_tiles = 0;
    a.sub_splits = 1;
    a.P2 = nullptr;
    a.unit_grid = 1;
    a.k_inline = 0;
    a.pos_raw = nullptr;
    for (int d = 0; d < TBK_MAX_DIM; ++d) a.k_val[d] = 0.0;
    if (tbk_hk_gemv_path(m, nk)) {
        int slices;
        size_t lds;
        gemv_plan(m, nk, &slices, &lds);
        const size_t per_split = (size_t)nk * a.ncol_pad * 2 * sizeof(double);
        if (m->h_k_inline != nullptr && nk == 1 && d_A == nullptr && tbk_hk_inline_phases(m, 1)) {
            a.k_inline = 1;
            for (int d = 0; d < m->dim; ++d) a.k_val[d] = m->h_k_inline[d];
            a.pos_raw = m->d_pos_inline;
        }
        TBK_ARG(d_A != nullptr || (tbk_hk_inline_phases(m, nk) && (d_k != nullptr || a.k_inline)), "phase rows missing");
        TBK_ARG(convention != 1 || mode == HK_TRI || d_pos != nullptr || (a.k_inline && a.pos_raw != nullptr), "convention 1 needs the orbital phases");
        if (nk == 1 && d_A == nullptr && a.ncol_pad <= 256 && m->k2 <= 4096) {
            const int strip = (int)(((m->k2 / 2 + 3) / 4 * 2 + 15) / 16 * 16);
            const size_t lds_tiny = ((size_t)4 * strip + 4 * 64 * 2) * sizeof(double);
            const dim3 grid_tiny((unsigned)(a.ncol_pad / 64));
            StageTimer t(m, TBK_T_HK);
            if (mode == HK_TRI)
                hipLaunchKernelGGL((hk_tiny_kernel<HK_TRI, 2>), grid_tiny, dim3(256), lds_tiny, m->stream, a, strip);
            else if (convention == 1)
                hipLaunchKernelGGL((hk_tiny_kernel<HK_FULL, 1>), grid_tiny, dim3(256), lds_tiny, m->stream, a, strip);
            else
                hipLaunchKernelGGL((hk_tiny_kernel<HK_FULL, 2>), grid_tiny, dim3(256), lds_tiny, m->stream, a, strip);
            TBK_HIP(hipGetLastError());
            return TBK_OK;
        }
        TBK_CHECK(m->ws_part.reserve(per_split * slices));
        a.P = m->ws_part.as<double>();
        a.splits = slices;
        a.p_rows = nk;
        StageTimer t(m, TBK_T_HK);
        if (mode == HK_TRI) {
            TBK_HIP((launch_gemv<HK_TRI, 2>(m, a, lds, m->stream)));
        } else if (convention == 1) {
            TBK_HIP((launch_gemv<HK_FULL, 1>(m, a, lds, m->stream)));
        } else {
            TBK_HIP((launch_gemv<HK_FULL, 2>(m, a, lds, m->stream)));
        }
        return TBK_OK;
    }
    const int n_stage = (int)(m->k2 / TBK_BK);
    const int tiles = a.mt_count * a.nt_count;
    if (tiles < 2 * m->n_cu && n_stage >= 16) {
        int splits = std::min((1280 + tiles / 2) / tiles, n_stage / 4);
        const size_t per_split = (size_t)nk_pad * a.ncol_pad * 2 * sizeof(double);
        splits = (int)std::min<size_t>((size_t)splits, (size_t(512) << 20) / per_split);
        if (splits > 1) {
            TBK_CHECK(m->ws_part.reserve(per_split * splits));
            a.P = m->ws_part.as<double>();
            a.splits = splits;
            a.p_rows = nk_pad;
        }
    }
    StageTimer t(m, TBK_T_HK);
    if (mode == HK_TRI) {
        TBK_CHECK((launch<HK_TRI, 2>(m, a, grid)));
    } else if (convention == 1) {
        TBK_CHECK((launch<HK_FULL, 1>(m, a, grid)));
    } else {
        TBK_CHECK((launch<HK_FULL, 2>(m, a, grid)));
    }
    return TBK_OK;
}

int tbk_launch_hk_dense_lines(tbk_model* m, const double* d_A, int64_t n_lines, int line_len, int64_t b_stride,
                              double* d_H) {
    if (n_lines == 0) return TBK_OK;
    TBK_ARG(line_len >= 1 && line_len <= TBK_BM, "a mesh line must fit one k tile");
    HkArgs a;
    a.A = d_A;
    a.Bt = m->d_B;
    a.colmap = m->d_colmap;
    a.kpts = nullptr;
    a.R = m->d_R;
    a.n_r = m->n_r;
    a.pos = nullptr;
    a.H = d_H;
    a.k2 = m->k2;
    a.nk = n_lines * line_len;
    a.nk_pad = TBK_BM;
    a.ncol_pad = m->ncol_pad;
    a.n_orb = m->n_orb;
    a.dim = m->dim;
    a.mt_count = (int)n_lines;
    a.nt_count = m->ncol_pad / TBK_BNP;
    a.P = nullptr;
    a.splits = 1;
    a.p_rows = 0;
    a.a_tile_stride = 0;
    a.b_tile_stride = b_stride;
    a.rows_per_tile = line_len;
    a.block_offset = 0;
    a.p_tiles = 0;
    a.sub_splits = 1;
    a.P2 = nullptr;
    a.unit_grid = 1;
    int grid;
    if (a.mt_count >= 32) {
        a.xcd_rows = 4;
        grid = ((a.mt_count + 7) / 8) * a.nt_count * 8;
    } else {
        a.xcd_rows = 0;
        grid = a.mt_count * a.nt_count;
    }
    StageTimer t(m, TBK_T_HK);
    TBK_CHECK((launch<HK_TRI, 2>(m, a, grid)));
    return TBK_OK;
}
```

### tbmodels_amd/csrc/tbk_internal.h

```cpp
#pragma once

#include <hip/hip_runtime.h>
#include <rocblas/rocblas.h>

#include <atomic>
#include <cstdlib>
#include <cstdint>
#include <cstdio>
#include <functional>
#include <mutex>
#include <string>
#include <vector>

#include "tbk.h"

constexpr int TBK_BM = 128;
constexpr int TBK_BNP = 64;
constexpr int TBK_BK = 16;
constexpr int TBK_CT = 16;
constexpr int TBK_MAX_DIM = 8;

constexpr int32_t TBK_SLOT_PAIR = 0x8000;

void tbk_set_error(const char* fmt, ...);

#define TBK_HIP(expr)                                                                             \
    do {                                                                                          \
        hipError_t e_ = (expr);                                                                   \
        if (e_ != hipSuccess) {                                                                   \
            tbk_set_error("%s failed: %s (%s:%d)", #expr, hipGetErrorString(e_), __FILE__,        \
                          __LINE__);                                                              \
            return (e_ == hipErrorOutOfMemory) ? TBK_ERR_MEMORY : TBK_ERR_DEVICE;                 \
        }                                                                                         \
    } while (0)

#define TBK_ROCBLAS(expr)                                                                         \
    do {                                                                                          \
        rocblas_status s_ = (expr);                                                               \
        if (s_ != rocblas_status_success) {                                                       \
            tbk_set_error("%s failed: rocblas_status %d (%s:%d)", #expr, (int)s_, __FILE__,       \
                          __LINE__);                                                              \
            return (s_ == rocblas_status_memory_error) ? TBK_ERR_MEMORY : TBK_ERR_DEVICE;         \
        }                                                                                         \
    } while (0)

#define TBK_CHECK(expr)                                                                           \
    do {                                                                                          \
        int r_ = (expr);                                                                          \
        if (r_ != TBK_OK) return r_;                                                              \
    } while (0)

#define TBK_LOCK(m) std::lock_guard<std::recursive_mutex> tbk_lock_((m)->mu)

#define TBK_ARG(cond, msg)                                                                        \
    do {                                                                                          \
        if (!(cond)) {                                                                            \
            tbk_set_error("invalid argument: %s", msg);                                           \
            return TBK_ERR_ARGUMENT;                                                              \
        }                                                                                         \
    } while (0)


constexpr int TBK_MAX_DEVICES = 64;

using tbk_flag_row = std::atomic<bool>[TBK_MAX_DEVICES];
inline hipError_t tbk_raise_lds_limit(const void* kernel, int bytes, tbk_flag_row& done) {
    int dev = 0;
    hipError_t e = hipGetDevice(&dev);
    if (e != hipSuccess) return e;
    if (dev >= 0 && dev < TBK_MAX_DEVICES && done[dev].load(std::memory_order_acquire)) return hipSuccess;
    e = hipFuncSetAttribute(kernel, hipFuncAttributeMaxDynamicSharedMemorySize, bytes);
    if (e == hipSuccess && dev >= 0 && dev < TBK_MAX_DEVICES) done[dev].store(true, std::memory_order_release);
    return e;
}

struct DevBuf {
    void* ptr = nullptr;
    size_t bytes = 0;
    int reserve(size_t want);
    void release();
    template <class T>
    T* as() const {
        return static_cast<T*>(ptr);
    }
};

struct EventPair {
    hipEvent_t start, stop;
    int stage;
};

struct tbk_fold_plan_t {
    bool built = false;
    int dim = 0;
    int64_t n_r = 0;
    int64_t n_rho = 0, n_rho_pad = 0, k2 = 0;
    int capacity = 0;
    std::vector<int32_t> h_R2;
    int32_t* d_R2 = nullptr;
    int64_t* d_lptr = nullptr;
    int32_t* d_lrec = nullptr;
    int32_t* d_rcomp = nullptr;
    double* d_B2 = nullptr;
    double* d_table = nullptr;
    int64_t table_entries = 0;
    tbk_fold_plan_t* sub = nullptr;
};

struct tbk_fold_saved_t {
    int dim;
    int64_t n_r, n_r_pad, k2;
    int32_t* d_R;
    double* d_B;
};

struct tbk_model {
    std::recursive_mutex mu;
    int device = 0;
    int64_t call_nk = 0;
    int n_cu = 256;
    int dim = 0;
    int n_orb = 0;
    int64_t n_r = 0;
    bool sparse = false;
    bool kdotp = false;

    int64_t n_r_pad = 0;
    int64_t k2 = 0;
    int ncol = 0;
    int ncol_pad = 0;
    int32_t* d_R = nullptr;
    int32_t* d_colmap = nullptr;
    int32_t* d_powers = nullptr;

    double* d_B = nullptr;

    int64_t nnz_rec = 0;
    int64_t* d_cptr = nullptr;
    int32_t* d_rec_r = nullptr;
    double* d_rec_v = nullptr;
    int sched_kt = 0;
    int64_t sched_steps = 0;
    int64_t* d_sptr = nullptr;
    int32_t* d_srec_r = nullptr;
    double* d_srec_v = nullptr;

    int64_t staged_bytes = 0;

    std::vector<int32_t> h_R;
    tbk_fold_plan_t fold[TBK_MAX_DIM];
    bool fold_enabled = true;
    int64_t counters[TBK_CNT_COUNT] = {0, 0, 0, 0};

    int eigensolver = TBK_EIG_AUTO;
    int64_t k_chunk = 0;
    bool timing = false;

    hipStream_t stream = nullptr;
    hipStream_t stream_eig = nullptr;
    hipStream_t stream_ql = nullptr;
    hipStream_t stream_xl[3] = {nullptr, nullptr, nullptr};
    hipEvent_t ev_xl[4] = {nullptr, nullptr, nullptr, nullptr};
    hipEvent_t ev_hk[2] = {nullptr, nullptr};
    hipEvent_t ev_tri[2] = {nullptr, nullptr};
    hipEvent_t ev_out[2] = {nullptr, nullptr};
    hipEvent_t ev_ql[2] = {nullptr, nullptr};
    hipEvent_t ev_sync = nullptr;
    rocblas_handle blas = nullptr;
    DevBuf ws_phase;
    DevBuf ws_H;
    DevBuf ws_H2;
    DevBuf ws_E;
    DevBuf ws_E2;
    DevBuf ws_info;
    DevBuf ws_k;
    DevBuf ws_pos;
    DevBuf ws_orb;
    DevBuf ws_out;
    DevBuf ws_out2;
    DevBuf ws_flag;
    void* h_stage = nullptr;
    size_t h_stage_bytes = 0;
    DevBuf ws_part;
    DevBuf ws_kfold;
    DevBuf ws_kline;
    DevBuf ws_band;
    DevBuf ws_bandmat[2];
    const double* h_k_inline = nullptr;
    const double* d_pos_inline = nullptr;
    std::vector<double> pos_cache;
    DevBuf ws_posraw;
    DevBuf ws_xl;
    std::function<int(int64_t c0, int64_t nkc, hipEvent_t done)> chunk_done;
    std::vector<EventPair> events;
    double t_ms[TBK_T_COUNT] = {0, 0, 0, 0};
    int64_t t_n[TBK_T_COUNT] = {0, 0, 0, 0};
};

struct tbk_kdotp {
    tbk_model* core = nullptr;
};

void tbk_range_push(const char* name);
void tbk_range_pop();

struct StageTimer {
    tbk_model* m;
    EventPair ev;
    bool on;
    hipStream_t stream;
    StageTimer(tbk_model* m_, int stage, hipStream_t s = nullptr);
    ~StageTimer();
};

enum HkMode { HK_TRI = 0, HK_FULL = 1 };

int tbk_launch_phase(tbk_model* m, const double* d_k, int64_t nk, int64_t nk_pad, double* d_A);
int tbk_launch_orbital_phases(tbk_model* m, const double* d_k, const double* d_pos, int64_t nk, double* d_orb);
int tbk_launch_monomials(hipStream_t s, const int32_t* d_powers, int dim, int64_t n_p,
                         int64_t n_p_pad, const double* d_k, int64_t nk, int64_t nk_pad,
                         double* d_A);

int tbk_stage_dense(tbk_model* m, const double* d_hop_raw);
int tbk_stage_kdotp(tbk_model* m, const double* d_coeff_raw);

int tbk_launch_hk_dense(tbk_model* m, const double* d_A, int64_t nk, int64_t nk_pad, int mode,
                        int convention, const double* d_k, const double* d_pos, double* d_H);

int tbk_launch_hk_dense_lines(tbk_model* m, const double* d_A, int64_t n_lines, int line_len, int64_t b_stride, double* d_H);

int tbk_launch_hk_csr(tbk_model* m, const double* d_A, int64_t nk, int64_t nk_pad, int mode,
                      int convention, const double* d_k, const double* d_pos, double* d_H);

int tbk_csr_tile_kpoints(int64_t n_r);
void tbk_csr_schedule(int ncol, int kt, const std::vector<int64_t>& cptr, const std::vector<int32_t>& rec_r, const std::vector<double>& rec_v,
                      std::vector<int64_t>& sptr, std::vector<int32_t>& srec_r, std::vector<double>& srec_v);

int tbk_eig_batched(tbk_model* m, double* d_H, int64_t nk, double* d_E);

bool tbk_eig_stream_supported(int n);
int tbk_launch_tridiag_stream(tbk_model* m, hipStream_t s, double* d_H, int64_t nk, double* d_de, int method = 0);
bool tbk_hk_inline_phases(const tbk_model* m, int64_t nk);
bool tbk_hk_gemv_path(const tbk_model* m, int64_t nk);
int tbk_launch_bisect(tbk_model* m, hipStream_t s, const double* d_de, int64_t nk, double* d_E);
size_t tbk_eig_scratch_per_k(const tbk_model* m);
int tbk_band_xl_reserve(tbk_model* m, int64_t max_nk);

bool tbk_eig_band_supported(int n);
bool tbk_eig_band_preferred(int n);
size_t tbk_band_scratch_per_matrix(int n);
size_t tbk_band_bytes_per_matrix(int n);
size_t tbk_band_xl_buffer_per_matrix(int n);
bool tbk_eig_two_stage(const tbk_model* m);
int tbk_launch_band_reduce(tbk_model* m, hipStream_t s, double* d_H, int64_t nk, void* d_vw, void* d_band,
                           double* d_de_fused = nullptr);
bool tbk_band_fused(int n);
bool tbk_band_split(const tbk_model* m, int64_t nk);
bool tbk_band_xl_grouped(int n, int64_t nk);
int tbk_launch_band_chase(tbk_model* m, hipStream_t s, const void* d_band, int64_t nk, double* d_de);

bool tbk_eig_small_supported(int n);
int tbk_launch_tridiag(tbk_model* m, hipStream_t s, double* d_H, int64_t nk, double* d_de);
bool tbk_eig_reg128_supported(int n);
int tbk_launch_tridiag_reg128(hipStream_t s, double* d_H, int n, int64_t nk, double* d_D, double* d_E, int64_t h_stride, int ldd, int off);
int tbk_launch_tridiag_tail64(hipStream_t s, double* d_H, int64_t nk, double* d_D, double* d_E, int n_full, int64_t call_nk);
int tbk_launch_ql(tbk_model* m, hipStream_t s, const double* d_de, int64_t nk, double* d_E, bool beside_ql = false);

int tbk_fold_choose(tbk_model* m, const double* h_k, int64_t nk, std::vector<int64_t>& run_starts);
int tbk_fold_group_size();
int tbk_fold_group(tbk_model* m, tbk_fold_plan_t& plan, const double* h_kf, int n_g, int slot0);
int tbk_fold_lines(tbk_model* m, tbk_fold_plan_t& plan, const double* d_kf, int64_t stride, int n_lines, int slot0 = 0);
int tbk_fold_enter(tbk_model* m, tbk_fold_plan_t& plan, int slot, tbk_fold_saved_t& saved);
void tbk_fold_leave(tbk_model* m, const tbk_fold_saved_t& saved);
int tbk_fold_drop_component(tbk_model* m, const double* d_k, int dim, int f, int64_t nk, double* d_k2);
int tbk_fold_subplan(tbk_model* m, tbk_fold_plan_t& parent, int f2, int capacity, tbk_fold_plan_t** out);
void tbk_fold_release(tbk_model* m);
int64_t tbk_fold_min_run();

int tbk_run_mfma_f64_peak(double* tflops);
```

### tbmodels_amd/csrc/tbk_phase.hip

```cpp

#include "tbk_internal.h"

namespace {

__global__ void __launch_bounds__(256)
phase_rows_kernel(const double* __restrict__ k, const int32_t* __restrict__ R, int dim, int64_t nk,
                  int64_t nk_pad, int64_t n_r, double* __restrict__ A) {
    const int64_t kidx = (int64_t)blockIdx.x * blockDim.x + threadIdx.x;
    const int64_t r = blockIdx.y;
    if (kidx >= nk_pad) return;
    double c = 0.0, s = 0.0;
    if (kidx < nk && r < n_r) {
        double dot = 0.0;
        for (int d = 0; d < dim; ++d)
            dot = fma(k[kidx * dim + d], (double)R[r * dim + d], dot);
        sincospi(2.0 * dot, &s, &c);
    }
    A[(2 * r) * nk_pad + kidx] = c;
    A[(2 * r + 1) * nk_pad + kidx] = s;
}

__global__ void __launch_bounds__(256)
monomial_rows_kernel(const double* __restrict__ k, const int32_t* __restrict__ powers, int dim,
                     int64_t nk, int64_t nk_pad, int64_t n_p, double* __restrict__ A) {
    const int64_t kidx = (int64_t)blockIdx.x * blockDim.x + threadIdx.x;
    const int64_t p = blockIdx.y;
    if (kidx >= nk_pad) return;
    double v = 0.0;
    if (kidx < nk && p < n_p) {
        v = 1.0;
        for (int d = 0; d < dim; ++d) {
            const double x = k[kidx * dim + d];
            const int e = powers[p * dim + d];
            double acc = 1.0;
            for (int t = 0; t < e; ++t) acc *= x;
            v *= acc;
        }
    }
    A[p * nk_pad + kidx] = v;
}

__global__ void __launch_bounds__(256)
orbital_phase_kernel(const double* __restrict__ k, const double* __restrict__ pos, int dim, int64_t nk,
                     int n_orb, double* __restrict__ orb) {
    const int64_t idx = (int64_t)blockIdx.x * blockDim.x + threadIdx.x;
    if (idx >= nk * n_orb) return;
    const int64_t kq = idx / n_orb;
    const int p = (int)(idx % n_orb);
    double dot = 0.0;
    for (int d = 0; d < dim; ++d) dot = fma(k[kq * dim + d], pos[p * dim + d], dot);
    double s, c;
    sincospi(2.0 * dot, &s, &c);
    orb[2 * idx] = c;
    orb[2 * idx + 1] = s;
}

}

int tbk_launch_orbital_phases(tbk_model* m, const double* d_k, const double* d_pos, int64_t nk, double* d_orb) {
    if (nk == 0) return TBK_OK;
    const int64_t total = nk * m->n_orb;
    hipLaunchKernelGGL(orbital_phase_kernel, dim3((unsigned)((total + 255) / 256)), dim3(256), 0, m->stream, d_k,
                       d_pos, m->dim, nk, m->n_orb, d_orb);
    TBK_HIP(hipGetLastError());
    return TBK_OK;
}

int tbk_launch_phase(tbk_model* m, const double* d_k, int64_t nk, int64_t nk_pad, double* d_A) {
    if (m->n_r_pad == 0 || nk_pad == 0) return TBK_OK;
    StageTimer t(m, TBK_T_PHASE);
    dim3 grid((unsigned)((nk_pad + 255) / 256), (unsigned)m->n_r_pad);
    hipLaunchKernelGGL(phase_rows_kernel, grid, dim3(256), 0, m->stream, d_k, m->d_R, m->dim, nk,
                       nk_pad, m->n_r, d_A);
    TBK_HIP(hipGetLastError());
    return TBK_OK;
}

int tbk_launch_monomials(hipStream_t s, const int32_t* d_powers, int dim, int64_t n_p,
                         int64_t n_p_pad, const double* d_k, int64_t nk, int64_t nk_pad,
                         double* d_A) {
    if (n_p_pad == 0 || nk_pad == 0) return TBK_OK;
    dim3 grid((unsigned)((nk_pad + 255) / 256), (unsigned)n_p_pad);
    hipLaunchKernelGGL(monomial_rows_kernel, grid, dim3(256), 0, s, d_k, d_powers, dim, nk, nk_pad,
                       n_p, d_A);
    TBK_HIP(hipGetLastError());
    return TBK_OK;
}
```

### tbmodels_amd/csrc/tbk_stage.hip

```cpp

#include "tbk_internal.h"

namespace {

__global__ void __launch_bounds__(256)
stage_dense_kernel(const double* __restrict__ hop, const int32_t* __restrict__ colmap, int n_orb,
                   int64_t n_r, int ncol_pad, double* __restrict__ Bt) {
    const int e = blockIdx.x * blockDim.x + threadIdx.x;
    const int64_t r = blockIdx.y;
    if (e >= ncol_pad || r >= n_r) return;
    const int32_t ij = colmap[e];
    if (ij < 0) return;
    const int i = ij >> 16, j = ij & 0x7fff;
    const double* blk = hop + (size_t)r * n_orb * n_orb * 2;
    const size_t tiles = ncol_pad / TBK_CT;
    const size_t base0 = (((size_t)(2 * r) * tiles + e / TBK_CT) * 2) * TBK_CT + e % TBK_CT;
    const size_t base1 = (((size_t)(2 * r + 1) * tiles + e / TBK_CT) * 2) * TBK_CT + e % TBK_CT;
    if (ij & TBK_SLOT_PAIR) {
        const double hr = blk[((size_t)i * n_orb + i) * 2], hi = blk[((size_t)i * n_orb + i) * 2 + 1];
        const double gr = blk[((size_t)j * n_orb + j) * 2], gi = blk[((size_t)j * n_orb + j) * 2 + 1];
        Bt[base0] = hr + hr;
        Bt[base0 + TBK_CT] = gr + gr;
        Bt[base1] = -(hi + hi);
        Bt[base1 + TBK_CT] = -(gi + gi);
        return;
    }
    const double hr = blk[((size_t)i * n_orb + j) * 2], hi = blk[((size_t)i * n_orb + j) * 2 + 1];
    const double gr = blk[((size_t)j * n_orb + i) * 2], gi = blk[((size_t)j * n_orb + i) * 2 + 1];
    Bt[base0] = hr + gr;
    Bt[base0 + TBK_CT] = hi - gi;
    Bt[base1] = -(hi + gi);
    Bt[base1 + TBK_CT] = hr - gr;
}

__global__ void __launch_bounds__(256)
stage_kdotp_kernel(const double* __restrict__ coeff, const int32_t* __restrict__ colmap, int n_orb,
                   int64_t n_p, int ncol_pad, double* __restrict__ Bt) {
    const int e = blockIdx.x * blockDim.x + threadIdx.x;
    const int64_t p = blockIdx.y;
    if (e >= ncol_pad || p >= n_p) return;
    const int32_t ij = colmap[e];
    if (ij < 0) return;
    const int i = ij >> 16, j = ij & 0xffff;
    const double* blk = coeff + (size_t)p * n_orb * n_orb * 2;
    const size_t tiles = ncol_pad / TBK_CT;
    const size_t base = (((size_t)p * tiles + e / TBK_CT) * 2) * TBK_CT + e % TBK_CT;
    Bt[base] = blk[((size_t)i * n_orb + j) * 2];
    Bt[base + TBK_CT] = blk[((size_t)i * n_orb + j) * 2 + 1];
}

}

int tbk_stage_dense(tbk_model* m, const double* d_hop_raw) {
    const size_t bytes = (size_t)m->k2 * m->ncol_pad * 2 * sizeof(double);
    if (bytes == 0) return TBK_OK;
    TBK_HIP(hipMalloc((void**)&m->d_B, bytes));
    m->staged_bytes += (int64_t)bytes;
    TBK_HIP(hipMemsetAsync(m->d_B, 0, bytes, m->stream));
    if (m->n_r > 0) {
        TBK_ARG(m->n_r <= 65535, "more than 65535 lattice vectors");
        dim3 grid((m->ncol_pad + 255) / 256, (unsigned)m->n_r);
        hipLaunchKernelGGL(stage_dense_kernel, grid, dim3(256), 0, m->stream, d_hop_raw, m->d_colmap,
                           m->n_orb, m->n_r, m->ncol_pad, m->d_B);
        TBK_HIP(hipGetLastError());
    }
    return TBK_OK;
}

int tbk_stage_kdotp(tbk_model* m, const double* d_coeff_raw) {
    const size_t bytes = (size_t)m->k2 * m->ncol_pad * 2 * sizeof(double);
    if (bytes == 0) return TBK_OK;
    TBK_HIP(hipMalloc((void**)&m->d_B, bytes));
    m->staged_bytes += (int64_t)bytes;
    TBK_HIP(hipMemsetAsync(m->d_B, 0, bytes, m->stream));
    if (m->n_r > 0) {
        TBK_ARG(m->n_r <= 65535, "more than 65535 Taylor coefficients");
        dim3 grid((m->ncol_pad + 255) / 256, (unsigned)m->n_r);
        hipLaunchKernelGGL(stage_kdotp_kernel, grid, dim3(256), 0, m->stream, d_coeff_raw,
                           m->d_colmap, m->n_orb, m->n_r, m->ncol_pad, m->d_B);
        TBK_HIP(hipGetLastError());
    }
    return TBK_OK;
}
```

Baseline: 991,200 k-points/s.

## Add one-level Strassen path for dense H(k) phase-by-hopping GEMM

Adds a Strassen 2x2 block decomposition for the dense H(k) GEMM. The seven B-side operand combinations are prestaged at model creation, the phase kernel writes the seven A-side combinations, one split kernel computes the seven half-size products, and a finish kernel combines them into the H slots. The aim is to cut the f64 matrix-multiply flops by about one eighth. In exchange it adds extra memory traffic for staged operands and partial products, an extra launch, a smaller chunk size, and slightly different floating-point rounding.

```diff
diff --git a/include/tbk.h b/include/tbk.h
--- a/include/tbk.h
+++ b/include/tbk.h
@@ -25,7 +25,8 @@
     TBK_OPT_EIGENSOLVER = 1,
     TBK_OPT_K_CHUNK = 2,
     TBK_OPT_TIMING = 3,
-    TBK_OPT_FOLD = 4
+    TBK_OPT_FOLD = 4,
+    TBK_OPT_STRASSEN = 5
 };
 
 const char* tbk_version(void);
@@ -46,7 +47,8 @@
                    int* is_sparse, int64_t* staged_bytes);
 enum { TBK_CNT_EIGENVAL_CALLS = 0, TBK_CNT_FOLDED_CALLS = 1, TBK_CNT_FOLDED_KPOINTS = 2,
        TBK_CNT_LIBRARY_CALLS = 3,
-       TBK_CNT_COUNT = 4 };
+       TBK_CNT_STRASSEN_LAUNCHES = 4,
+       TBK_CNT_COUNT = 5 };
 int tbk_model_counter(tbk_model* m, int counter, int64_t* value);
 
 
diff --git a/tbmodels_amd/_lib.py b/tbmodels_amd/_lib.py
--- a/tbmodels_amd/_lib.py
+++ b/tbmodels_amd/_lib.py
@@ -15,9 +15,9 @@
 TBK_ERR_NO_CONVERGENCE = 5
 
 TBK_EIG_AUTO, TBK_EIG_WAVE, TBK_EIG_ROCSOLVER = 0, 1, 2
-TBK_OPT_EIGENSOLVER, TBK_OPT_K_CHUNK, TBK_OPT_TIMING, TBK_OPT_FOLD = 1, 2, 3, 4
+TBK_OPT_EIGENSOLVER, TBK_OPT_K_CHUNK, TBK_OPT_TIMING, TBK_OPT_FOLD, TBK_OPT_STRASSEN = 1, 2, 3, 4, 5
 TBK_REDUCE_AUTO, TBK_REDUCE_ONE_STAGE, TBK_REDUCE_TWO_STAGE = 0, 1, 2
-TBK_CNT_EIGENVAL_CALLS, TBK_CNT_FOLDED_CALLS, TBK_CNT_FOLDED_KPOINTS, TBK_CNT_LIBRARY_CALLS = 0, 1, 2, 3
+TBK_CNT_EIGENVAL_CALLS, TBK_CNT_FOLDED_CALLS, TBK_CNT_FOLDED_KPOINTS, TBK_CNT_LIBRARY_CALLS, TBK_CNT_STRASSEN_LAUNCHES = 0, 1, 2, 3, 4
 TBK_T_PHASE, TBK_T_HK, TBK_T_EIG, TBK_T_QL, TBK_T_COUNT = 0, 1, 2, 3, 4
 STAGE_NAMES = ("phase", "hk", "eig", "ql")
 
diff --git a/tbmodels_amd/csrc/tbk_api.hip b/tbmodels_amd/csrc/tbk_api.hip
--- a/tbmodels_amd/csrc/tbk_api.hip
+++ b/tbmodels_amd/csrc/tbk_api.hip
@@ -146,10 +146,11 @@
     m->dim = dim;
     m->n_orb = n_orb;
     m->n_r = n_r;
-    m->k2 = round_up(n_r * k_rows_per_r, TBK_BK);
+    const bool strassen = pair_diagonal && k_rows_per_r == 2 && tbk_strassen_model(false, false, n_r);
+    m->k2 = round_up(n_r * k_rows_per_r, strassen ? 2 * TBK_BK : TBK_BK);
     m->n_r_pad = m->k2 / k_rows_per_r;
     m->ncol = (int)(pair_diagonal ? (int64_t)n_orb * (n_orb - 1) / 2 + (n_orb + 1) / 2 : (int64_t)n_orb * (n_orb + 1) / 2);
-    m->ncol_pad = (int)round_up(m->ncol, TBK_BNP);
+    m->ncol_pad = (int)round_up(m->ncol, strassen ? 2 * TBK_BNP : TBK_BNP);
 
     int rc = TBK_OK;
     auto fail = [&](int code) {
@@ -233,6 +234,7 @@
             TBK_HIP(hipMemcpyAsync(d_raw, hop, raw_bytes, hipMemcpyHostToDevice, m->stream));
         }
         TBK_CHECK(tbk_stage_dense(m, d_raw));
+        TBK_CHECK(tbk_stage_strassen(m));
         TBK_HIP(hipStreamSynchronize(m->stream));
         return TBK_OK;
     }();
@@ -352,7 +354,7 @@
     if (m->h_stage) (void)hipHostFree(m->h_stage);
     for (hipStream_t st : streams)
         if (st) (void)hipStreamDestroy(st);
-    void* ptrs[] = {m->d_R, m->d_colmap, m->d_B, m->d_cptr, m->d_rec_r, m->d_rec_v, m->d_powers, m->d_sptr, m->d_srec_r, m->d_srec_v};
+    void* ptrs[] = {m->d_R, m->d_colmap, m->d_B, m->d_Bs, m->d_cptr, m->d_rec_r, m->d_rec_v, m->d_powers, m->d_sptr, m->d_srec_r, m->d_srec_v};
     for (void* p : ptrs)
         if (p) (void)hipFree(p);
     DevBuf* bufs[] = {&m->ws_phase, &m->ws_H, &m->ws_E,   &m->ws_E2,
@@ -380,6 +382,9 @@
         case TBK_OPT_FOLD:
             m->fold_enabled = value != 0;
             return TBK_OK;
+        case TBK_OPT_STRASSEN:
+            m->strassen = value != 0;
+            return TBK_OK;
         default:
             tbk_set_error("unknown option %d", option);
             return TBK_ERR_ARGUMENT;
@@ -406,13 +411,18 @@
     size_t free_b = 0, total_b = 0;
     if (hipMemGetInfo(&free_b, &total_b) != hipSuccess) free_b = size_t(8) << 30;
     free_b += m->ws_H.bytes + m->ws_H2.bytes + m->ws_phase.bytes + m->ws_band.bytes + m->ws_bandmat[0].bytes + m->ws_bandmat[1].bytes +
-              m->ws_E.bytes + m->ws_xl.bytes;
+              m->ws_E.bytes + m->ws_xl.bytes + m->ws_part.bytes;
     const bool mid = n > 64 && n <= 256;
     int64_t budget = std::min<int64_t>((int64_t)(free_b / 4), int64_t(mid ? 64 : n > 64 ? 24 : 6) << 30);
     int64_t chunk = budget / per_k / TBK_BM * TBK_BM;
     int64_t cap = mid ? 131072 : 32768;
     if (n < 64) cap *= std::min<int64_t>(32, (64 / n) * (64 / n));
     chunk = std::max<int64_t>(TBK_BM, std::min<int64_t>(chunk, cap));
+    if (tbk_hk_strassen(m, std::min(chunk, nk))) {
+        const int64_t per_k_s = per_k + m->k2 * 8 * 3 / 4 + (int64_t)m->ncol_pad * 16 * 7 / 4;
+        const int64_t fit = (int64_t)(free_b / 4) / per_k_s / TBK_BM * TBK_BM;
+        chunk = std::max<int64_t>(TBK_BM, std::min(chunk, fit));
+    }
     if (m->k_chunk > 0) chunk = round_up(m->k_chunk, TBK_BM);
     else if (chunk >= 4096) chunk = chunk / 4096 * 4096;
     return std::min(chunk, round_up(nk, TBK_BM));
@@ -421,6 +431,7 @@
 static inline int64_t phase_ld(int64_t nk) { return round_up(nk, TBK_BM); }
 
 static int fill_rows(tbk_model* m, const double* d_k, int64_t nk, int64_t nk_pad, double* d_A) {
+    if (tbk_hk_strassen(m, nk)) return tbk_launch_phase_strassen(m, d_k, nk, d_A);
     if (m->kdotp)
         return tbk_launch_monomials(m->stream, m->d_powers, m->dim, m->n_r, m->k2, d_k, nk, nk_pad, d_A);
     return tbk_launch_phase(m, d_k, nk, nk_pad, d_A);
@@ -448,7 +459,7 @@
     for (int64_t c0 = 0; c0 < nk; c0 += chunk) {
         const int64_t nkc = std::min(chunk, nk - c0);
         const int64_t nk_pad = phase_ld(nkc);
-        TBK_CHECK(m->ws_phase.reserve((size_t)std::max<int64_t>(m->k2, 1) * nk_pad * sizeof(double)));
+        TBK_CHECK(m->ws_phase.reserve((size_t)tbk_phase_doubles(m, nkc, nk_pad) * sizeof(double)));
         double* d_A = m->ws_phase.as<double>();
         const double* kc = d_k + c0 * m->dim;
         const bool own_rows = tbk_hk_inline_phases(m, nkc);
@@ -522,7 +533,7 @@
     const auto prepare_rows = [&](int64_t c0, int64_t nkc) -> int {
         if (tbk_hk_inline_phases(m, nkc)) return TBK_OK;
         const int64_t nk_pad = phase_ld(nkc);
-        TBK_CHECK(m->ws_phase.reserve((size_t)std::max<int64_t>(m->k2, 1) * nk_pad * sizeof(double)));
+        TBK_CHECK(m->ws_phase.reserve((size_t)tbk_phase_doubles(m, nkc, nk_pad) * sizeof(double)));
         TBK_CHECK(fill_rows(m, d_k + c0 * m->dim, nkc, nk_pad, m->ws_phase.as<double>()));
         rows_ready_for = c0;
         return TBK_OK;
@@ -649,7 +660,7 @@
 
     auto piece_plane = [&](int64_t lo, int64_t hi, double* d_Hp) -> int {
         const int64_t len = hi - lo, nk_pad = phase_ld(len);
-        TBK_CHECK(m->ws_phase.reserve((size_t)std::max<int64_t>(m->k2, 1) * nk_pad * sizeof(double)));
+        TBK_CHECK(m->ws_phase.reserve((size_t)tbk_phase_doubles(m, len, nk_pad) * sizeof(double)));
         TBK_CHECK(fill_rows(m, d_k2 + lo * (dim - 1), len, nk_pad, m->ws_phase.as<double>()));
         return build_h(m, m->ws_phase.as<double>(), len, nk_pad, HK_TRI, 2, d_k2 + lo * (dim - 1), nullptr, d_Hp);
     };
@@ -847,7 +858,7 @@
     for (int64_t c0 = 0; c0 < nk; c0 += chunk) {
         const int64_t nkc = std::min(chunk, nk - c0);
         const int64_t nk_pad = phase_ld(nkc);
-        TBK_CHECK(m->ws_phase.reserve((size_t)std::max<int64_t>(m->k2, 1) * nk_pad * sizeof(double)));
+        TBK_CHECK(m->ws_phase.reserve((size_t)tbk_phase_doubles(m, nkc, nk_pad) * sizeof(double)));
         TBK_CHECK(m->ws_H.reserve((size_t)nkc * nn2 * sizeof(double)));
         double* d_A = m->ws_phase.as<double>();
         double* d_H = m->ws_H.as<double>();
diff --git a/tbmodels_amd/csrc/tbk_hk_dense.hip b/tbmodels_amd/csrc/tbk_hk_dense.hip
--- a/tbmodels_amd/csrc/tbk_hk_dense.hip
+++ b/tbmodels_amd/csrc/tbk_hk_dense.hip
@@ -40,6 +40,8 @@
     int splits;
     int unit_grid;
     int64_t p_rows;
+    int products;
+    int64_t a_prod_stride, b_prod_stride;
     int64_t a_tile_stride;
     int64_t b_tile_stride;
     int rows_per_tile;
@@ -151,8 +153,13 @@
 #pragma unroll
             for (int p = 0; p < 2; ++p) acc[i][j][p] = (d4){0.0, 0.0, 0.0, 0.0};
 
+    const double* opA = a.A;
+    const double* opB = a.Bt;
     int s_begin = 0, n_stage = (int)(a.k2 / TBK_BK);
-    if (SPLIT) {
+    if (SPLIT && a.products) {
+        opA += split_y * a.a_prod_stride;
+        opB += split_y * a.b_prod_stride;
+    } else if (SPLIT) {
         const int per = (n_stage + a.splits - 1) / a.splits;
         s_begin = min(split_y * per, n_stage);
         n_stage = min(s_begin + per, n_stage);
@@ -166,8 +173,8 @@
     const uint32_t lane_bytes = (uint32_t)lane * 16u;
     const int64_t ldgA = a.nk_pad * (int64_t)sizeof(double);
     const int64_t ldgB = (int64_t)a.ncol_pad * 2 * (int64_t)sizeof(double);
-    const char* rowA = reinterpret_cast<const char*>(a.A + (int64_t)mt_idx * a.a_tile_stride) + ((int64_t)s_begin * TBK_BK + wave) * ldgA;
-    const char* rowB = reinterpret_cast<const char*>(a.Bt + (int64_t)mt_idx * a.b_tile_stride + n0 * 2) + ((int64_t)s_begin * TBK_BK + wave) * ldgB;
+    const char* rowA = reinterpret_cast<const char*>(opA + (int64_t)mt_idx * a.a_tile_stride) + ((int64_t)s_begin * TBK_BK + wave) * ldgA;
+    const char* rowB = reinterpret_cast<const char*>(opB + (int64_t)mt_idx * a.b_tile_stride + n0 * 2) + ((int64_t)s_begin * TBK_BK + wave) * ldgB;
     auto issue_stage = [&](auto bufc) {
         constexpr int buf = decltype(bufc)::value;
         double* sA = smem + buf * STAGE_DOUBLES + wave * LDA;
@@ -257,7 +264,7 @@
     for (int j = 0; j < 2; ++j) {
         const int e = (int)n0 + (wn * 2 + j) * 16 + l15;
         const int32_t ij = a.colmap[e];
-        if (ij < 0) continue;
+        if (ij < 0 && !(SPLIT && a.products)) continue;
 #pragma unroll
         for (int i = 0; i < 4; ++i) {
 #pragma unroll
@@ -453,6 +460,31 @@
         im += v[1];
     }
     store_slot<MODE, CONV>(a, kq, ij, re, im);
+}
+
+template <int MODE, int CONV>
+__global__ void __launch_bounds__(256) hk_strassen_finish_kernel(const HkArgs a, int64_t mh) {
+    const int half = a.ncol_pad / 2;
+    const int64_t idx = (int64_t)blockIdx.x * 256 + threadIdx.x;
+    const int e = (int)(idx % half);
+    const int64_t kq = idx / half;
+    if (kq >= mh) return;
+    const size_t blk = (size_t)mh * half;
+    const d2* mp = reinterpret_cast<const d2*>(a.P) + (size_t)kq * half + e;
+    const d2 m1 = mp[0], m2 = mp[blk], m3 = mp[2 * blk], m4 = mp[3 * blk], m5 = mp[4 * blk], m6 = mp[5 * blk], m7 = mp[6 * blk];
+    const d2 c11 = ((m1 + m4) - m5) + m7;
+    const d2 c12 = m3 + m5;
+    const d2 c21 = m2 + m4;
+    const d2 c22 = ((m1 - m2) + m3) + m6;
+    const int32_t ij0 = a.colmap[e], ij1 = a.colmap[e + half];
+    if (kq < a.nk) {
+        if (ij0 >= 0) store_slot<MODE, CONV>(a, kq, ij0, c11[0], c11[1]);
+        if (ij1 >= 0) store_slot<MODE, CONV>(a, kq, ij1, c12[0], c12[1]);
+    }
+    if (kq + mh < a.nk) {
+        if (ij0 >= 0) store_slot<MODE, CONV>(a, kq + mh, ij0, c21[0], c21[1]);
+        if (ij1 >= 0) store_slot<MODE, CONV>(a, kq + mh, ij1, c22[0], c22[1]);
+    }
 }
 
 template <int MODE, int CONV>
@@ -621,6 +653,49 @@
     return TBK_OK;
 }
 
+template <int MODE, int CONV>
+int launch_strassen(tbk_model* m, const HkArgs& a0) {
+    hipStream_t s = m->stream;
+    const size_t lds = 2 * STAGE_DOUBLES * sizeof(double);
+    static std::atomic<bool> raised[TBK_MAX_DEVICES] = {};
+    TBK_HIP(tbk_raise_lds_limit(reinterpret_cast<const void*>(&hk_dense_kernel<HK_TRI, 2, true>), 160 * 1024, raised));
+    const int64_t mh = tbk_strassen_mh(a0.nk);
+    const int half = a0.ncol_pad / 2;
+    HkArgs a = a0;
+    a.Bt = m->d_Bs;
+    a.k2 = m->k2 / 2;
+    a.nk = mh;
+    a.nk_pad = mh;
+    a.ncol_pad = half;
+    a.mt_count = (int)(mh / TBK_BM);
+    a.nt_count = half / TBK_BNP;
+    int grid;
+    if (a.mt_count >= 32) {
+        a.xcd_rows = 4;
+        grid = ((a.mt_count + 7) / 8) * a.nt_count * 8;
+    } else {
+        a.xcd_rows = 0;
+        grid = a.mt_count * a.nt_count;
+    }
+    a.products = 1;
+    a.splits = 7;
+    a.unit_grid = grid;
+    a.p_rows = mh;
+    a.a_prod_stride = a.k2 * mh;
+    a.b_prod_stride = a.k2 * half * 2;
+    TBK_CHECK(m->ws_part.reserve((size_t)7 * mh * half * 2 * sizeof(double)));
+    a.P = m->ws_part.as<double>();
+    hipLaunchKernelGGL((hk_dense_kernel<HK_TRI, 2, true>), dim3(7 * grid), dim3(256), lds, s, a);
+    TBK_HIP(hipGetLastError());
+    HkArgs f = a0;
+    f.P = a.P;
+    const int64_t threads = mh * half;
+    hipLaunchKernelGGL((hk_strassen_finish_kernel<MODE, CONV>), dim3((unsigned)((threads + 255) / 256)), dim3(256), 0, s, f, mh);
+    TBK_HIP(hipGetLastError());
+    m->counters[TBK_CNT_STRASSEN_LAUNCHES] += 1;
+    return TBK_OK;
+}
+
 int gemv_nkv(int64_t nk) {
     int nkv = 1;
     while (nkv < std::min<int64_t>(nk, 32)) nkv *= 2;
@@ -655,6 +730,18 @@
     *lds_out = lds;
 }
 
+}
+
+bool tbk_hk_strassen(const tbk_model* m, int64_t nk) {
+    if (!m->strassen || m->d_Bs == nullptr || m->d_B != m->bs_src || m->sparse || m->kdotp) return false;
+    if (m->n_r_pad < TBK_STRASSEN_MIN_NR || nk < TBK_STRASSEN_MIN_NK || tbk_hk_gemv_path(m, nk)) return false;
+    const int64_t tiles = (nk + TBK_BM - 1) / TBK_BM * (m->ncol_pad / TBK_BNP);
+    return tiles >= 2 * m->n_cu;
+}
+
+int64_t tbk_phase_doubles(const tbk_model* m, int64_t nk, int64_t nk_pad) {
+    if (tbk_hk_strassen(m, nk)) return 7 * (m->k2 / 2) * tbk_strassen_mh(nk);
+    return std::max<int64_t>(m->k2, 1) * nk_pad;
 }
 
 bool tbk_hk_inline_phases(const tbk_model* m, int64_t nk) {
@@ -703,6 +790,8 @@
     a.P = nullptr;
     a.splits = 1;
     a.p_rows = 0;
+    a.products = 0;
+    a.a_prod_stride = a.b_prod_stride = 0;
     a.a_tile_stride = TBK_BM;
     a.b_tile_stride = 0;
     a.rows_per_tile = TBK_BM;
@@ -751,6 +840,17 @@
             TBK_HIP((launch_gemv<HK_FULL, 1>(m, a, lds, m->stream)));
         } else {
             TBK_HIP((launch_gemv<HK_FULL, 2>(m, a, lds, m->stream)));
+        }
+        return TBK_OK;
+    }
+    if (d_A != nullptr && tbk_hk_strassen(m, nk)) {
+        StageTimer t(m, TBK_T_HK);
+        if (mode == HK_TRI) {
+            TBK_CHECK((launch_strassen<HK_TRI, 2>(m, a)));
+        } else if (convention == 1) {
+            TBK_CHECK((launch_strassen<HK_FULL, 1>(m, a)));
+        } else {
+            TBK_CHECK((launch_strassen<HK_FULL, 2>(m, a)));
         }
         return TBK_OK;
     }
@@ -802,6 +902,8 @@
     a.P = nullptr;
     a.splits = 1;
     a.p_rows = 0;
+    a.products = 0;
+    a.a_prod_stride = a.b_prod_stride = 0;
     a.a_tile_stride = 0;
     a.b_tile_stride = b_stride;
     a.rows_per_tile = line_len;
diff --git a/tbmodels_amd/csrc/tbk_internal.h b/tbmodels_amd/csrc/tbk_internal.h
--- a/tbmodels_amd/csrc/tbk_internal.h
+++ b/tbmodels_amd/csrc/tbk_internal.h
@@ -134,6 +134,8 @@
     int32_t* d_powers = nullptr;
 
     double* d_B = nullptr;
+    double* d_Bs = nullptr;
+    const double* bs_src = nullptr;
 
     int64_t nnz_rec = 0;
     int64_t* d_cptr = nullptr;
@@ -150,7 +152,8 @@
     std::vector<int32_t> h_R;
     tbk_fold_plan_t fold[TBK_MAX_DIM];
     bool fold_enabled = true;
-    int64_t counters[TBK_CNT_COUNT] = {0, 0, 0, 0};
+    bool strassen = true;
+    int64_t counters[TBK_CNT_COUNT] = {0, 0, 0, 0, 0};
 
     int eigensolver = TBK_EIG_AUTO;
     int64_t k_chunk = 0;
@@ -215,6 +218,14 @@
 
 enum HkMode { HK_TRI = 0, HK_FULL = 1 };
 
+constexpr int64_t TBK_STRASSEN_MIN_NR = 1024;
+constexpr int64_t TBK_STRASSEN_MIN_NK = 8192;
+inline bool tbk_strassen_model(bool sparse, bool kdotp, int64_t n_r) { return !sparse && !kdotp && n_r >= TBK_STRASSEN_MIN_NR; }
+bool tbk_hk_strassen(const tbk_model* m, int64_t nk);
+inline int64_t tbk_strassen_mh(int64_t nk) { return (((nk + 1) / 2) + TBK_BM - 1) / TBK_BM * TBK_BM; }
+int64_t tbk_phase_doubles(const tbk_model* m, int64_t nk, int64_t nk_pad);
+
+int tbk_launch_phase_strassen(tbk_model* m, const double* d_k, int64_t nk, double* d_As);
 int tbk_launch_phase(tbk_model* m, const double* d_k, int64_t nk, int64_t nk_pad, double* d_A);
 int tbk_launch_orbital_phases(tbk_model* m, const double* d_k, const double* d_pos, int64_t nk, double* d_orb);
 int tbk_launch_monomials(hipStream_t s, const int32_t* d_powers, int dim, int64_t n_p,
@@ -223,6 +234,7 @@
 
 int tbk_stage_dense(tbk_model* m, const double* d_hop_raw);
 int tbk_stage_kdotp(tbk_model* m, const double* d_coeff_raw);
+int tbk_stage_strassen(tbk_model* m);
 
 int tbk_launch_hk_dense(tbk_model* m, const double* d_A, int64_t nk, int64_t nk_pad, int mode,
                         int convention, const double* d_k, const double* d_pos, double* d_H);
diff --git a/tbmodels_amd/csrc/tbk_phase.hip b/tbmodels_amd/csrc/tbk_phase.hip
--- a/tbmodels_amd/csrc/tbk_phase.hip
+++ b/tbmodels_amd/csrc/tbk_phase.hip
@@ -18,6 +18,41 @@
     }
     A[(2 * r) * nk_pad + kidx] = c;
     A[(2 * r + 1) * nk_pad + kidx] = s;
+}
+
+__global__ void __launch_bounds__(256)
+phase_rows_strassen_kernel(const double* __restrict__ k, const int32_t* __restrict__ R, int dim, int64_t nk, int64_t mh,
+                           int64_t n_r, int64_t rh, double* __restrict__ As) {
+    const int64_t kq = (int64_t)blockIdx.x * blockDim.x + threadIdx.x;
+    const int64_t r = blockIdx.y;
+    if (kq >= mh) return;
+    double c[2][2], s[2][2];
+#pragma unroll
+    for (int a = 0; a < 2; ++a)
+#pragma unroll
+        for (int b = 0; b < 2; ++b) {
+            const int64_t kidx = kq + a * mh, rr = r + b * rh;
+            c[a][b] = 0.0;
+            s[a][b] = 0.0;
+            if (kidx < nk && rr < n_r) {
+                double dot = 0.0;
+                for (int d = 0; d < dim; ++d) dot = fma(k[kidx * dim + d], (double)R[rr * dim + d], dot);
+                sincospi(2.0 * dot, &s[a][b], &c[a][b]);
+            }
+        }
+    const size_t blk = (size_t)2 * rh * mh;
+#pragma unroll
+    for (int t = 0; t < 2; ++t) {
+        const double(&v)[2][2] = t == 0 ? c : s;
+        double* row = As + (size_t)(2 * r + t) * mh + kq;
+        row[0 * blk] = v[0][0] + v[1][1];
+        row[1 * blk] = v[1][0] + v[1][1];
+        row[2 * blk] = v[0][0];
+        row[3 * blk] = v[1][1];
+        row[4 * blk] = v[0][0] + v[0][1];
+        row[5 * blk] = v[1][0] - v[0][0];
+        row[6 * blk] = v[0][1] - v[1][1];
+    }
 }
 
 __global__ void __launch_bounds__(256)
@@ -76,6 +111,15 @@
     return TBK_OK;
 }
 
+int tbk_launch_phase_strassen(tbk_model* m, const double* d_k, int64_t nk, double* d_As) {
+    const int64_t mh = tbk_strassen_mh(nk), rh = m->n_r_pad / 2;
+    StageTimer t(m, TBK_T_PHASE);
+    dim3 grid((unsigned)((mh + 255) / 256), (unsigned)rh);
+    hipLaunchKernelGGL(phase_rows_strassen_kernel, grid, dim3(256), 0, m->stream, d_k, m->d_R, m->dim, nk, mh, m->n_r, rh, d_As);
+    TBK_HIP(hipGetLastError());
+    return TBK_OK;
+}
+
 int tbk_launch_monomials(hipStream_t s, const int32_t* d_powers, int dim, int64_t n_p,
                          int64_t n_p_pad, const double* d_k, int64_t nk, int64_t nk_pad,
                          double* d_A) {
diff --git a/tbmodels_amd/csrc/tbk_stage.hip b/tbmodels_amd/csrc/tbk_stage.hip
--- a/tbmodels_amd/csrc/tbk_stage.hip
+++ b/tbmodels_amd/csrc/tbk_stage.hip
@@ -49,6 +49,40 @@
     Bt[base + TBK_CT] = blk[((size_t)i * n_orb + j) * 2 + 1];
 }
 
+__global__ void __launch_bounds__(256)
+stage_strassen_kernel(const double* __restrict__ Bt, int64_t kh, int ncol_pad, double* __restrict__ Bs) {
+    const int j = blockIdx.x * blockDim.x + threadIdx.x;
+    const int64_t kk = blockIdx.y;
+    if (j >= ncol_pad) return;
+    const size_t row = (size_t)2 * ncol_pad;
+    const double b11 = Bt[kk * row + j], b12 = Bt[kk * row + ncol_pad + j];
+    const double b21 = Bt[(kk + kh) * row + j], b22 = Bt[(kk + kh) * row + ncol_pad + j];
+    const size_t blk = (size_t)kh * ncol_pad, o = kk * (size_t)ncol_pad + j;
+    Bs[0 * blk + o] = b11 + b22;
+    Bs[1 * blk + o] = b11;
+    Bs[2 * blk + o] = b12 - b22;
+    Bs[3 * blk + o] = b21 - b11;
+    Bs[4 * blk + o] = b22;
+    Bs[5 * blk + o] = b11 + b12;
+    Bs[6 * blk + o] = b21 + b22;
+}
+
+}
+
+int tbk_stage_strassen(tbk_model* m) {
+    if (!tbk_strassen_model(m->sparse, m->kdotp, m->n_r) || m->d_B == nullptr) return TBK_OK;
+    const int64_t kh = m->k2 / 2;
+    if (kh % TBK_BK != 0 || m->ncol_pad % (2 * TBK_BNP) != 0 || kh > 65535) return TBK_OK;
+    const size_t bytes = (size_t)7 * kh * m->ncol_pad * sizeof(double);
+    size_t free_b = 0, total_b = 0;
+    if (hipMemGetInfo(&free_b, &total_b) != hipSuccess || bytes > free_b / 4) return TBK_OK;
+    TBK_HIP(hipMalloc((void**)&m->d_Bs, bytes));
+    m->staged_bytes += (int64_t)bytes;
+    m->bs_src = m->d_B;
+    dim3 grid((m->ncol_pad + 255) / 256, (unsigned)kh);
+    hipLaunchKernelGGL(stage_strassen_kernel, grid, dim3(256), 0, m->stream, m->d_B, kh, m->ncol_pad, m->d_Bs);
+    TBK_HIP(hipGetLastError());
+    return TBK_OK;
 }
 
 int tbk_stage_dense(tbk_model* m, const double* d_hop_raw) {
```

Result: faster. 1.073 million k-points/s (median of 6 runs) (+8.3%).
